# W298/Surtr

Hardware: AMD Instinct MI355X
Metric: fragments/sec (higher is better)
Workload: dtype f32

## Files before the change

### surtr_amd/csrc/prep_sorted.h

```cpp
#pragma once
#include "wave_clip.h"

#define PS_NEVER 0x7Fu
#ifndef SURTR_PS_NB
#define SURTR_PS_NB 896u
#endif
#ifndef SURTR_SPH_FAN
#define SURTR_SPH_FAN 8u
#endif

namespace surtr {

struct SortedRings
{
    const SRow* row_s; const uint32_t* iperm;
    const float4* bsph2; const float4* bsph3;
};

__device__ __forceinline__ uint32_t ps_sphere_fc(const Shared& sh, const uint32_t F, const float4 sp, const uint32_t k0, uint32_t& kstop)
{
    const float mag = fabsf(sp.x) + fabsf(sp.y) + fabsf(sp.z) + sp.w;
    for (uint32_t k = k0; k < F; ++k)
    {
        const float4 mk = sh.pmar[k];
// ... 311 lines not shown
    __syncthreads();
    for (uint32_t id = tid; id < n; id += G)
    {
        const uint32_t v = orig[id] & 0xFFFFu;
        const float4 pr = in.posr_s[orig[id] >> 16];
        T.pos[3 * id] = pr.x; T.pos[3 * id + 1] = pr.y; T.pos[3 * id + 2] = pr.z;
        const uint32_t deg = T.llen[id];
        const int32_t* r = in.nbr + in.loff[v];
        uint16_t* d = T.ring + T.loff[id];
        for (uint32_t j0 = 0; j0 < deg; j0 += 8)
        {
            int32_t u[8];
#pragma unroll
            for (int q = 0; q < 8; ++q) u[q] = (j0 + q < deg) ? r[j0 + q] : -1;
#pragma unroll
            for (int q = 0; q < 8; ++q) if (u[q] >= 0) d[j0 + q] = (uint16_t)ps_newid(bmask, bblk, (uint32_t)u[q], InLds::SENT);
        }
    }
    STAMP(2);
    __syncthreads();
    uint32_t maxb = 0;
    for (uint32_t k = 0; k < F; ++k) maxb = sh.pw[k] > maxb ? sh.pw[k] : maxb;
    maxb_out = maxb;
    T.nS = n; T.nLive = n; T.hUsed = hsum;
}

struct RecLayout { uint32_t hist, zhist, bst, grec, gpos, total; };
__host__ __device__ static inline RecLayout rec_layout(uint32_t F, uint32_t n)
{
    auto up = [](uint32_t b) { return (b + 15u) & ~15u; };
    const uint32_t nn = (n + 15u) & ~15u;
    RecLayout L;
    L.hist = 0; L.zhist = up(4u * F); L.bst = L.zhist + up(4u * F); L.grec = L.bst + up(4u * (F + 2u)); L.gpos = L.grec + 16u * nn;
    L.total = L.gpos + 16u * nn;
    return L;
}

__device__ __attribute__((always_inline)) inline void prepass_emit_records(const SolidIn in, const uint32_t F, Shared& sh, const unsigned long long* bmask, const uint2* bblk,
                                                                           const uint32_t* klist, uint32_t* orig, uint8_t* fcb, uint16_t* sid16, uint32_t* cnt,
                                                                           char* img, const uint32_t n, uint32_t& ncut_out, uint32_t& maxb_out)
{
    const uint32_t tid = threadIdx.x, l = lane_id(), w = wave_id(), G = group_size(), nw = group_waves();
    const RecLayout lay = rec_layout(F, n);
    STAMP_DECL;
    for (uint32_t t = tid; t < n; t += G)
    {
        const uint32_t ke = klist[t], si = ke & 0xFFFFu;
        const uint32_t v = in.perm[si];
        const uint32_t id = ps_newid(bmask, bblk, v, 0u);
        orig[id] = v | (si << 16);
        fcb[id] = (uint8_t)((ke >> 16) & 0x7Fu);
    }
    const uint32_t nsw = nw < 4u ? nw : 4u;
    uint32_t* wcnt = cnt;
    uint32_t* bst = cnt + 4u * (WC_MAXF + 2u);
    for (uint32_t k = tid; k < 4u * (WC_MAXF + 2u); k += G) wcnt[k] = 0u;
    __syncthreads();
    const unsigned long long lt = (1ull << l) - 1ull;
    const uint32_t nb = (n + SURTR_LANES - 1u) >> SURTR_LSH, nbw = (nb + nsw - 1u) / nsw;
    const uint32_t bb0 = w * nbw, bb1 = w < nsw ? (bb0 + nbw < nb ? bb0 + nbw : nb) : bb0;
    for (int pass = 0; pass < 2; ++pass)
    {
        for (uint32_t bb = bb0; bb < bb1; ++bb)
        {
            const uint32_t id = (bb << SURTR_LSH) + l;
            const bool valid = id < n;
            const uint32_t f = valid ? (uint32_t)fcb[id] : 0u;
            const uint32_t bk = (f == PS_NEVER || f > F) ? F : f;
            unsigned long long todo = __ballot(valid);
            uint32_t s = 0;
            while (todo)
            {
                const uint32_t leader = (uint32_t)__builtin_ctzll(todo);
                const uint32_t k0 = lane_bcast(bk, leader);
                const unsigned long long same = __ballot(valid && bk == k0);
                uint32_t base = 0;
                if (l == leader) { base = wcnt[w * (WC_MAXF + 2u) + k0]; wcnt[w * (WC_MAXF + 2u) + k0] = base + wc_popc64(same); }
                base = lane_bcast(base, leader);
                if (valid && bk == k0) s = base + wc_popc64(same & lt);
                todo &= ~same;
            }
            if (valid && pass == 1) sid16[id] = (uint16_t)s;
        }
        if (pass == 1) break;
        __syncthreads();
        if (w == 0u)
        {
            uint32_t carry = 0;
            for (uint32_t k0 = 0; k0 <= F; k0 += SURTR_LANES)
            {
                const uint32_t k = k0 + l;
                uint32_t c = 0;
                if (k <= F) for (uint32_t q = 0; q < nsw; ++q) c += wcnt[q * (WC_MAXF + 2u) + k];
                const uint32_t inc = wave_incl_scan2(make_uint2(c, 0u)).x;
                if (k <= F)
                {
                    uint32_t at = carry + inc - c;
                    bst[k] = at;
                    for (uint32_t q = 0; q < nsw; ++q) { const uint32_t cq = wcnt[q * (WC_MAXF + 2u) + k]; wcnt[q * (WC_MAXF + 2u) + k] = at; at += cq; }
                }
                carry += lane_bcast(inc, SURTR_LANES - 1u);
            }
            if (l == 0u) bst[F + 1u] = carry;
        }
        __syncthreads();
    }
    __syncthreads();
    STAMP(2);
    WcW4* grec = (WcW4*)(img + lay.grec);
    float4* gpos = (float4*)(img + lay.gpos);
    for (uint32_t id = tid; id < n; id += G)
    {
        const uint32_t vi = orig[id], v = vi & 0xFFFFu;
        const uint32_t f = fcb[id];
        const uint32_t len = in.llen[v];
        const int32_t* r = in.nbr + in.loff[v];
        const uint32_t s = sid16[id];
        const float4 pr = in.posr_s[vi >> 16];
        int32_t u[7]; uint32_t e[7];
#pragma unroll
        for (uint32_t q = 0; q < 7u; ++q) u[q] = r[q < len ? q : 0u];
#pragma unroll
        for (uint32_t q = 0; q < 7u; ++q) e[q] = ps_newid(bmask, bblk, (uint32_t)u[q], 0xFFFFFFFFu);
#pragma unroll
        for (uint32_t q = 0; q < 7u; ++q) e[q] = q >= len ? WC_NONE : (e[q] == 0xFFFFFFFFu ? WC_SENT : (uint32_t)sid16[e[q]]);
        WcW4 wr;
        wr.a = e[0] | (e[1] << 16); wr.b = e[2] | (e[3] << 16); wr.c = e[4] | (e[5] << 16);
        wr.d = e[6] | (((f == PS_NEVER ? SURTR_NEVER : f) | (len << 8)) << 16);
        grec[s] = wr;
        gpos[s] = make_float4(pr.x, pr.y, pr.z, __uint_as_float(id));
    }
    prepass_finish_hist(F, sh);
    uint32_t* hs = (uint32_t*)(img + lay.hist); uint32_t* zs = (uint32_t*)(img + lay.zhist); uint32_t* bs = (uint32_t*)(img + lay.bst);
    for (uint32_t k = tid; k < F; k += G) { hs[k] = sh.hist[k]; zs[k] = sh.zhist[k]; }
    for (uint32_t k = tid; k <= F + 1u; k += G) bs[k] = bst[k];
    uint32_t ncut = 0, maxb = 0;
    for (uint32_t k = 0; k < F; ++k) { const uint32_t c = bst[k + 1u] - bst[k]; ncut += c != 0u ? 1u : 0u; maxb = c > maxb ? c : maxb; }
    ncut_out = ncut; maxb_out = maxb;
    STAMP(74);
}

template <class LT>
__device__ __attribute__((always_inline)) inline int wc_attach(LT& W, const uint32_t* hist, const uint32_t* zhist, const uint32_t* bst, const uint32_t F, const uint32_t n,
                                                               unsigned long long& zmask, WcCtr& ctr, uint32_t* __restrict__ why)
{
    const uint32_t tid = threadIdx.x;
    ctr.ac = 0u; ctr.sc = 0u;
    zmask = 0ull;
    if (F > WC_MAXF || n == 0u || n >= WC_MAXN) WC_RET(1);
    WSTAMP_DECL;
    for (uint32_t k = tid; k < F; k += group_size()) { W.hist[k] = hist[k]; W.zhist[k] = zhist[k]; }
    for (uint32_t k = tid; k <= F + 1u; k += group_size()) W.bst[k] = bst[k];
    if (tid == 0u) { W.zm[0] = 0u; W.zm[1] = 0u; for (int q = 0; q < 6; ++q) (&W.fl[0][0])[q] = 0u; }
    __syncthreads();
    WSTAMP(1);
    WCOUNT(16, 1); WCOUNT(17, n);
    return 0;
}

}
```

### surtr_amd/csrc/surtr_ctx.h

```cpp
#pragma once
#include <algorithm>
#include <chrono>
#include <cstdint>
#include <cstdlib>
#include <string>
#include <vector>

#include "../../include/surtr_hip.h"
#include "clip_core.h"

using namespace surtr;

struct PairRec
{
    uint32_t cv_off, cv_n, ch_off, ch_n;
    uint32_t mv_off, mv_n, mh_off, mh_n;
    uint32_t ni, isl_off;
    uint32_t status;
    uint32_t img_fmt, img_off, img_n, img_h, img_pc;
    uint32_t cv_bad;
};

enum { IMG_NONE = 0,
       IMG_NARROW = 1,
       IMG_WIDE = 2,
       IMG_EMPTY = 3,
       IMG_REC = 4 };

struct ImgLayout { uint32_t hist, zhist, nzero, mask, loff, llen, comp, ring, pos, total; };
__host__ __device__ static inline ImgLayout img_layout(uint32_t F, uint32_t nbV, uint32_t n, uint32_t hsum, uint32_t posCap = 0)
{
    auto up = [](uint32_t b) { return (b + 15u) & ~15u; };
    ImgLayout L;
    L.hist = 0; L.zhist = up(4u * F); L.nzero = L.zhist + up(4u * F); L.mask = L.nzero + up(4u * F); L.loff = L.mask + up(8u * nbV);
    L.llen = L.loff + up(2u * n); L.comp = L.llen + up(n); L.ring = L.comp + up(n); L.pos = L.ring + up(2u * hsum);
    L.total = L.pos + up(12u * (n > posCap ? n : posCap));
    return L;
}

struct ImgArena { char* base; uint32_t cap16; };

struct PrepPool { char* base; size_t per_wg; uint32_t VMAX; };
static size_t prep_bytes_per_wg(uint32_t VMAX)
{
    auto r = [](size_t b) { return (b + 255) & ~(size_t)255; };
    return 2 * r((size_t)VMAX * 4) + r((size_t)(VMAX / SURTR_SB + 2) * 4) + 2 * r((size_t)(VMAX / SURTR_LANES + 2) * 8) +
           2 * r((size_t)VMAX + 64) +
           2 * r((size_t)VMAX * 4) +
           r((size_t)VMAX * 2 + 64);
}

struct FragRec
{
    int32_t cell, piece, island;
    uint32_t mv_off, mv_n, mh_off, mh_n;
    uint32_t cv_off, cv_n, ch_off, ch_n;
    uint32_t idx_off, idx_n;
    uint32_t o_mv, o_mh, o_cv, o_ch, o_idx;
};

struct Arena
{
    float* pos; uint32_t* loff; uint32_t* llen; int32_t* nbr; uint32_t* idx;
    uint2* isl;
    uint32_t capV, capH, capI, capIsl;
    uint32_t* cursors;
};

enum : uint32_t
{
    CUR_V = 0,
    CUR_H = 1,
    CUR_I = 2,
    CUR_ISL = 3,
    CUR_Q_CLIP = 4,
    CUR_STATUS = 5,
    CUR_Q_REFIT = 6,
    CUR_Q_FACES = 7,
    CUR_Q_CONVEX = 8,
    CUR_Q_PREP = 9,
    CUR_IMG = 10,
    CUR_Q_BIG = 11,
    CUR_Q_HALF = 12,
    CUR_Q_RETRY = 13,
    CUR_FLAGGED_FRAGS = 14,
    CUR_FLAGGED_PAIRS = 15,
    CUR_CLS_CLIP = 16,
    CUR_CLS_FRAG = 32,
    CUR_CLS_PREP = 48,
    CUR_CLS_HALF = 64,
    CUR_RETRY_N = CUR_CLS_HALF,
    CUR_CVX_RESUMED = 78,
    CUR_REFIT_RESUMED = 79,
    CUR_CVX_TOOK = 80,
    CUR_REFIT_TOOK = 82,
    CUR_BIG_QUOTA = 84,
    CUR_FACES2_N = 85,
    CUR_Q_FACES2 = 86,
    CUR_CVX_GAVE_UP = 87,
    CUR_REC_TOOK = 88,
    CUR_REC_HANDED = 89,
    CUR_LIT_TOO_LARGE = 90,
    CUR_REC_IMAGES = 91,
    CUR_SORTED_SEL = 92,
    CUR_REC_SPENT = 93,
    CUR_CATCH_CLIPPED = 94,
    CUR_UNREFITTED = 95,
    CUR_WC_WHY = 96,
    CUR_Q_CONVEX2 = 125,
    CUR_STATS_WORDS = 128,
    CUR_HO_PUSHED = 146,
    CUR_HO_STARTED = 147,
    CUR_HO_SIGNED_OFF = 148,
    CUR_HO_POLL_SLOT = 149,
    CUR_Q_CATCH = 150,
    CUR_Q_SWEEP = 151,
    CUR_HO_WORDS = 6,
    CUR_COUNT = 256
};
static_assert(CUR_V == 0 && CUR_H == 1 && CUR_I == 2 && CUR_ISL == 3 && CUR_STATUS == 5 && CUR_CLS_CLIP == 16 && CUR_CLS_FRAG == 32 &&
              CUR_CLS_PREP == 48 && CUR_CLS_HALF == 64 && CUR_REC_TOOK == 88 && CUR_REC_HANDED == 89 && CUR_LIT_TOO_LARGE == 90 &&
              CUR_UNREFITTED == 95 && CUR_WC_WHY == 96, "include/surtr_hip.h publishes these slots of surtr_queue_stats by number");
static_assert(CUR_STATS_WORDS <= CUR_COUNT && CUR_Q_SWEEP + 1 == CUR_HO_PUSHED + CUR_HO_WORDS && CUR_HO_PUSHED + CUR_HO_WORDS <= CUR_COUNT &&
              CUR_Q_FACES2 == CUR_FACES2_N + 1, "slot map");

struct alignas(16) SRow { uint32_t w[4]; };

struct Pieces
{
    const float* mpos; const uint32_t* mloff; const uint32_t* mllen; const int32_t* mnbr; const uint32_t* mvo; const uint8_t* mtri; const float* mrad;
    const uint32_t* mperm; const float4* mposr_s; const float4* mbsph; const uint32_t* mbo;
    const float* cpos; const uint32_t* cloff; const uint32_t* cllen; const int32_t* cnbr; const uint32_t* cvo; const uint8_t* ctri; const float* crad;
    const uint32_t* cperm; const float4* cposr_s; const float4* cbsph; const uint32_t* cbo;
    uint32_t n;
    const uint8_t* mdup; const uint8_t* cdup;
    const SRow* mrow_s; const uint32_t* miperm;
    const float4* mbsph2; const uint32_t* mbo2; const float4* mbsph3; const uint32_t* mbo3;
};

struct ScratchPool
{
    char* base; size_t per_wg;
    uint32_t CV, CH, VMAX;
};

struct Scratch
{
    float* pos;
    uint32_t* g_loff; uint32_t* g_llen; int8_t* g_comp; uint32_t* g_ring;
    uint32_t* g_succ; uint32_t* g_pred; uint32_t* g_pcnt;
    uint32_t* aux0; uint32_t* aux1; uint32_t* aux2; uint32_t* aux3;
    int8_t* g_gcomp;
    uint2* blk;
    unsigned long long* gmask; uint2* gblk;
    float* t_pos; uint32_t* t_loff; uint32_t* t_llen; int8_t* t_comp; uint32_t* t_ring;
    uint32_t CV, CH;
};

__device__ static Scratch carve(const ScratchPool& P, uint32_t wg)
{
    Scratch S;
    char* p = P.base + (size_t)wg * P.per_wg;
    auto take = [&](size_t bytes) { char* r = p; p += (bytes + 255) & ~(size_t)255; return r; };
    S.pos = (float*)take((size_t)P.CV * 12);
    S.g_loff = (uint32_t*)take((size_t)P.CV * 4);
    S.g_llen = (uint32_t*)take((size_t)P.CV * 4);
    S.g_comp = (int8_t*)take((size_t)P.CV);
    S.g_ring = (uint32_t*)take((size_t)P.CH * 4);
    S.g_succ = (uint32_t*)take((size_t)P.CV * 4);
    S.g_pred = (uint32_t*)take((size_t)P.CV * 4);
    S.g_pcnt = (uint32_t*)take((size_t)P.CV * 4);
    const size_t AV = P.CV > P.VMAX ? P.CV : P.VMAX;
    S.aux0 = (uint32_t*)take(AV * 4);
    S.aux1 = (uint32_t*)take((size_t)P.CV * 4);
    S.aux2 = (uint32_t*)take(AV * 4);
    S.aux3 = (uint32_t*)take((size_t)P.CV * 4);
    S.g_gcomp = (int8_t*)take((size_t)P.CV);
    S.blk = (uint2*)take((size_t)(P.CV / SURTR_LANES + 4) * 8);
    S.gmask = (unsigned long long*)take((size_t)(P.VMAX / SURTR_LANES + 2) * 8);
    S.gblk = (uint2*)take((size_t)(P.VMAX / SURTR_LANES + 2) * 8);
    S.t_pos = (float*)take((size_t)P.CV * 12); S.t_loff = (uint32_t*)take((size_t)P.CV * 4); S.t_llen = (uint32_t*)take((size_t)P.CV * 4);
    S.t_comp = (int8_t*)take((size_t)P.CV); S.t_ring = (uint32_t*)take((size_t)P.CH * 4);
    S.CV = P.CV; S.CH = P.CH;
    return S;
}

static size_t scratch_bytes_per_wg(uint32_t CV, uint32_t CH, uint32_t VMAX)
{
    auto r = [](size_t b) { return (b + 255) & ~(size_t)255; };
    return 2 * r((size_t)CV * 12) + 9 * r((size_t)CV * 4) + 2 * r((size_t)std::max(CV, VMAX) * 4) + 3 * r((size_t)CV) + 2 * r((size_t)CH * 4) + r((size_t)(CV / SURTR_LANES + 4) * 8) +
           2 * r((size_t)(VMAX / SURTR_LANES + 2) * 8);
}

struct FaceScratch
{
    int32_t* base; size_t per_wg; uint32_t HF;
};

struct surtr_ctx;

template <class T>
struct DevBuf
{
    T* p = nullptr;
    size_t cap = 0;
    DevBuf() = default;
    DevBuf(DevBuf&& o) noexcept : p(o.p), cap(o.cap) { o.p = nullptr; o.cap = 0; }
    DevBuf& operator=(DevBuf&& o) noexcept { if (this != &o) { reset(); p = o.p; cap = o.cap; o.p = nullptr; o.cap = 0; } return *this; }
    ~DevBuf() { reset(); }
    void reset() { if (p) (void)hipFree(p); p = nullptr; cap = 0; }
    operator T*() const { return p; }
    int grow(surtr_ctx* ctx, size_t need, size_t alloc = 0);
};

struct PieceSet
{
    DevBuf<float> pos; DevBuf<uint32_t> loff, llen; DevBuf<int32_t> nbr; DevBuf<uint32_t> vo; DevBuf<uint8_t> tri; DevBuf<float> rad;
    DevBuf<uint32_t> perm; DevBuf<float4> posr_s, bsph; DevBuf<uint32_t> bo;
    DevBuf<float> box; DevBuf<unsigned long long> key, key2; DevBuf<uint32_t> val;
    DevBuf<uint8_t> dup;
    DevBuf<uint32_t> iperm; DevBuf<SRow> row_s;
    DevBuf<float4> bsph2; DevBuf<uint32_t> bo2; DevBuf<float4> bsph3; DevBuf<uint32_t> bo3;
};

struct CellBuffers
{
    DevBuf<double> seeds; DevBuf<uint32_t> goff; DevBuf<char> slots; DevBuf<uint32_t> cfo, cvo;
    DevBuf<int32_t> gen; DevBuf<uint32_t> fvo; DevBuf<double> verts; DevBuf<uint32_t> heads;
    uint32_t n = 0, nf = 0, nfv = 0;
};

#define SURTR_LVS (SURTR_LV / 2u)
#define SURTR_LHS ((SURTR_LH * 11u / 24u) & ~7u)
#ifndef SURTR_HALF_ROOM
#define SURTR_HALF_ROOM 2u
#endif
__host__ __device__ static inline bool fits_half(uint32_t n, uint32_t h, uint32_t capVs) { return SURTR_HALF_ROOM * n <= capVs && SURTR_HALF_ROOM * h <= SURTR_LHS; }
static inline bool surtr_fits_half(uint32_t n, uint32_t h) { return fits_half(n, h, SURTR_LVS); }

struct surtr_ctx
{
    int device = 0;
    bool frags_of_pieces = false;
    uint32_t hw_wg = 512, hw_wg_faces = 1024, hw_wg_prep = 1792, hw_wg_big = 48, budget_vmax = 0xFFFFFFFFu, budget_hmax = 0xFFFFFFFFu;
    uint32_t max_wg = 512, max_wg_faces = 1024, max_wg_small = 2048, max_wg_lean = 3072, max_wg_prep = 1792, max_wg_half = 1024;
    DevBuf<uint32_t> d_hlist;
    uint32_t vmin = 0;
    ScratchPool pool_half{}; uint32_t n_wg_half = 0; DevBuf<char> pool_half_buf;
    bool half_on = false;
    PrepPool prep{nullptr, 0, 0}; uint32_t n_wg_prep = 0; DevBuf<char> prep_buf;
    ImgArena img{nullptr, 0}; DevBuf<char> img_buf;
    DevBuf<uint32_t> d_order;
    DevBuf<uint32_t> d_forder;
    bool wave_big = false;
    uint32_t n_wg_big = 48;
    hipStream_t stream2 = nullptr;
    hipStream_t stream3 = nullptr;
    hipEvent_t ev_prep = nullptr, ev_big = nullptr, ev_half = nullptr, ev_cvx = nullptr;
    uint32_t events_in_flight = 1;
    hipStream_t stream = nullptr;
    std::string err;
    uint32_t n_pieces = 0, vmax = 0, hmax = 0, cvmax = 0, chmax = 0;
// ... 252 lines not shown
```

### surtr_amd/csrc/surtr_hip.hip

```cpp
#include <algorithm>
#include <cmath>
#include <cstdio>
#include <cstdlib>
#include <cstring>
#include <string>
#include <type_traits>
#include <vector>

#include "surtr_ctx.h"
#include "small_clip.h"
#ifndef SC_RESUME
#define SC_RESUME 1
#endif
#include "literal_clip.h"
#include "wave_clip.h"
#include "prep_sorted.h"

template <uint32_t LV, uint32_t LH>
struct alignas(16) LdsTopoT
{
    static_assert(LV % 16 == 0 && LH % 8 == 0, "clip_image copies 16-byte words into these arrays");
    static constexpr uint32_t kLV = LV, kLH = LH;
    alignas(16) uint16_t loff[LV];
    alignas(16) uint8_t llen[LV];
// ... 1121 lines not shown
        }
        __syncthreads();
    }
    if (err == 0 && !gone) err = clip_global(min, F, S, sh, consume);
    __syncthreads();
    return finish_pair(A, pairs, p, rec, err);
}

template <bool HALF = false, class LT>
__device__ __attribute__((always_inline)) static inline void clip_pair_general(Shared& sh, LT& L, Scratch& S, const ScratchPool& pool, uint32_t wg, const Pieces& P,
                                       const float4* __restrict__ planes, const uint32_t* __restrict__ plane_off, uint32_t cell_begin,
                                       const Arena& A, const ImgArena& IA, PairRec* __restrict__ pairs, const uint2* __restrict__ pair_list,
                                       uint32_t* __restrict__ horder, const uint32_t p, PairRec rec)
{
    const uint32_t tid = threadIdx.x;
    const PairAt at = pair_where(p, pair_list, cell_begin, P.n);
    const uint32_t cell = at.cell, piece = at.piece;
    const uint32_t f0 = plane_off[cell], F = plane_off[cell + 1] - f0;
    for (uint32_t k = tid; k < F; k += group_size()) sh.planes[k] = planes[f0 + k];
    __syncthreads();
    SolidIn min = mesh_solid_in(P, piece);
    auto consume = [&](auto& T) -> int {
        if (T.nLive == 0) return 0;
        return park_mesh_islands(T, sh, A, rec);
    };
    if (P.mdup[piece] != 0 && min.nv <= SURTR_LITERAL_START_V)
    {
        if (HALF) { if (tid == 0) horder[atomicAdd(&A.cursors[CUR_RETRY_N], 1u)] = p; }
        else pair_global(P, piece, F, pool, wg, A, &sh, pairs, p, 1u);
        return;
    }
    int err;
    if (HALF)
    {
        if (rec.img_fmt == IMG_NARROW) err = clip_image<false>(IA.base + (size_t)rec.img_off * 16u, rec.img_n, rec.img_h, 0u, min, F, S, sh, L, consume);
        else err = clip_any<false>(min, F, S, sh, L, consume);
        __syncthreads();
        if (err == SURTR_OVERFLOW)
        {
            if (tid == 0) horder[atomicAdd(&A.cursors[CUR_RETRY_N], 1u)] = p;
            return;
        }
    }
    else
    {
        err = SURTR_OVERFLOW;
        if (rec.img_fmt == IMG_NARROW) err = clip_image<false>(IA.base + (size_t)rec.img_off * 16u, rec.img_n, rec.img_h, rec.img_pc, min, F, S, sh, L, consume);
        else if (rec.img_fmt != IMG_WIDE) err = clip_any<false>(min, F, S, sh, L, consume);
        __syncthreads();
        if (err == SURTR_OVERFLOW)
        {
            pair_global(P, piece, F, pool, wg, A, &sh, pairs, p, 0u);
            return;
        }
    }
    if (err == SURTR_E_TOPOLOGY && min.nv <= SURTR_LITERAL_MESH_V)
    {
        __syncthreads();
        if (HALF) { if (tid == 0) horder[atomicAdd(&A.cursors[CUR_RETRY_N], 1u)] = p; }
        else pair_global(P, piece, F, pool, wg, A, &sh, pairs, p, 1u);
        return;
    }
    finish_pair(A, pairs, p, rec, err);
}

template <bool HALF = false, class LT>
__device__ __attribute__((always_inline)) static inline void clip_pairs_body(Shared& sh, LT& L, const ScratchPool& pool, uint32_t wg, const Pieces& P, const float4* __restrict__ planes,
                                       const uint32_t* __restrict__ plane_off, uint32_t cell_begin, uint32_t n_pairs,
                                       const Arena& A, const ImgArena& IA, PairRec* __restrict__ pairs,
                                       const uint2* __restrict__ pair_list, const uint32_t* __restrict__ order,
                                       uint32_t* __restrict__ horder, int cls_hi, int cls_lo, uint32_t qcur)
{
    const uint32_t tid = threadIdx.x;
    Scratch S = carve(pool, wg);
#ifdef SURTR_STAMP
    const unsigned long long wg_t0 = __builtin_readcyclecounter();
#endif
    const int h_hi = HALF ? 6 : (cls_hi < 0 ? 0 : -1), h_lo = cls_hi < 0 ? 0 : 1;
    while (true)
    {
        __syncthreads();
        if (tid == 0)
        {
            uint32_t t = atomicAdd(&A.cursors[qcur], 1u), p = 0xFFFFFFFFu;
            if (!HALF) p = pair_of_ticket(A, order, n_pairs, t, CUR_CLS_CLIP, cls_hi, cls_lo);
            if (p == 0xFFFFFFFFu) p = pair_of_ticket(A, horder, n_pairs, t, CUR_CLS_HALF, h_hi, h_lo);
            sh.misc[7] = p;
        }
        __syncthreads();
        const uint32_t p = sh.misc[7];
        if (p >= n_pairs) break;
        PairRec rec = pairs[p];
        if (rec.cv_n == 0 || rec.status != 0) continue;
        if (rec.img_fmt == IMG_EMPTY) continue;
        if (rec.img_fmt == IMG_REC) rec.img_fmt = IMG_NONE;
#ifdef SURTR_STAMP
        const unsigned long long pair_t0 = __builtin_readcyclecounter();
        if (tid == 0) for (int q = 0; q < 16; ++q) sh.ph[q] = 0;
#endif
        clip_pair_general<HALF>(sh, L, S, pool, wg, P, planes, plane_off, cell_begin, A, IA, pairs, pair_list, horder, p, rec);
#ifdef SURTR_STAMP
        if (tid == 0) { const unsigned long long d = __builtin_readcyclecounter() - pair_t0; int bkt = 0; while ((d >> bkt) > 1 && bkt < 30) ++bkt; bkt = bkt < 16 ? 0 : bkt - 16; if (bkt > 9) bkt = 9; atomicAdd(&g_stamp[(cls_hi == 15 ? 51 : 21) + bkt], 1ull); }
#endif
    }
#ifdef SURTR_STAMP
    if (tid == 0) { const unsigned long long d = __builtin_readcyclecounter() - wg_t0; const int o = cls_hi == 15 ? 48 : 16; atomicAdd(&g_stamp[o], d); atomicMax(&g_stamp[o + 1], d); atomicAdd(&g_stamp[o + 2], 1ull); }
#endif
}

__global__ __launch_bounds__(SURTR_WG) __attribute__((amdgpu_waves_per_eu(2, 4))) void k_clip_pairs(Pieces P, const float4* __restrict__ planes,
                                                         const uint32_t* __restrict__ plane_off, uint32_t cell_begin,
                                                         uint32_t n_pairs,
                                                         ScratchPool pool, Arena A, ImgArena IA, PairRec* __restrict__ pairs,
                                                         const uint2* __restrict__ pair_list, const uint32_t* __restrict__ order,
                                                         uint32_t* __restrict__ horder, int cls_hi, int cls_lo, uint32_t qcur)
{
    __shared__ Shared sh;
    __shared__ LdsTopo L;
    clip_pairs_body(sh, L, pool, blockIdx.x, P, planes, plane_off, cell_begin, n_pairs, A, IA, pairs, pair_list, order, horder, cls_hi, cls_lo, qcur);
}

__global__ __launch_bounds__(SURTR_WGS) __attribute__((amdgpu_waves_per_eu(2, 4))) void k_clip_pairs_half(Pieces P, const float4* __restrict__ planes,
                                                         const uint32_t* __restrict__ plane_off, uint32_t cell_begin,
                                                         uint32_t n_pairs,
                                                         ScratchPool pool, Arena A, ImgArena IA, PairRec* __restrict__ pairs,
                                                         const uint2* __restrict__ pair_list, uint32_t* __restrict__ horder)
{
    __shared__ Shared sh;
    __shared__ LdsTopoHalf L;
    clip_pairs_body<true>(sh, L, pool, blockIdx.x, P, planes, plane_off, cell_begin, n_pairs, A, IA, pairs, pair_list, nullptr, horder, 6, 1, CUR_Q_HALF);
}

__global__ __launch_bounds__(SURTR_WG) void k_clip_pairs_big(Pieces P, const float4* __restrict__ planes,
                                                             const uint32_t* __restrict__ plane_off, uint32_t cell_begin,
                                                             uint32_t n_pairs,
                                                             ScratchPool pool, uint32_t wg_base, Arena A, ImgArena IA,
                                                             PairRec* __restrict__ pairs, const uint2* __restrict__ pair_list,
                                                             const uint32_t* __restrict__ order)
{
    __shared__ Shared sh;
    __shared__ LdsTopoBig L;
    clip_pairs_body(sh, L, pool, wg_base + blockIdx.x, P, planes, plane_off, cell_begin, n_pairs, A, IA, pairs, pair_list, order, nullptr, 15, 14, CUR_Q_BIG);
}

struct GenLds { Shared sh; LdsTopo L; };
struct GenLdsBig { Shared sh; LdsTopoBig L; };
template <class WL, class GL, bool FALLBACK = true, bool OLD_IMAGES = FALLBACK>
__device__ __attribute__((always_inline)) static inline void clip_pairs_wave_body(unsigned char* lds_raw, uint32_t wg, const Pieces& P, const float4* __restrict__ planes,
                                                         const uint32_t* __restrict__ plane_off, uint32_t cell_begin,
                                                         uint32_t n_pairs,
                                                         const ScratchPool& pool, const Arena& A, const ImgArena& IA, PairRec* __restrict__ pairs,
                                                         const uint2* __restrict__ pair_list, const uint32_t* __restrict__ order,
                                                         uint32_t* __restrict__ horder, int cls_hi, int cls_lo, uint32_t qcur, uint32_t walk0,
                                                         uint32_t* __restrict__ hlist, uint32_t cbase)
{
    WL& W = *reinterpret_cast<WL*>(lds_raw);
    GL& Gn = *reinterpret_cast<GL*>(lds_raw);
    const uint32_t tid = threadIdx.x;
    char* slot = pool.base + (size_t)wg * pool.per_wg;
    Scratch S{};
    if (FALLBACK) S = carve(pool, wg);
    if (!FALLBACK && tid == 0) atomicAdd(&A.cursors[CUR_HO_STARTED], 1u);
    while (true)
    {
        __syncthreads();
        if (tid == 0)
        {
            W.misc[7] = take_pair(A, order, n_pairs, qcur, cbase, cls_hi, cls_lo);
        }
        __syncthreads();
        const uint32_t p = W.misc[7];
        if (p >= n_pairs) break;
        PairRec rec = pairs[p];
        if (rec.cv_n == 0 || rec.status != 0) continue;
        if (rec.img_fmt == IMG_EMPTY) continue;
        const PairAt at = pair_where(p, pair_list, cell_begin, P.n);
        const uint32_t cell = at.cell, piece = at.piece;
        const uint32_t f0 = plane_off[cell], F = plane_off[cell + 1] - f0;
        int err = WC_BAIL;
        if ((rec.img_fmt == IMG_NARROW || rec.img_fmt == IMG_REC) && P.mdup[piece] == 0 && F <= WC_MAXF)
        {
            for (uint32_t k = tid; k < F; k += group_size()) W.planes[k] = planes[f0 + k];
            const uint32_t m0 = P.mvo[piece], V = P.mvo[piece + 1] - m0;
            const uint32_t nbV = (V + SURTR_LANES - 1u) >> SURTR_LSH;
            char* img = IA.base + (size_t)rec.img_off * 16u;
            unsigned long long zmask = 0ull;
            WcOut o{0u, 0u, 0u, 0u};
            WcCtr ctr{0u, 0u};
#ifdef SURTR_STAMP
            if (tid == 0) for (int q = 0; q < 32; ++q) W.ph[q] = 0ull;
#endif
            bool fits = false;
            WcGlob g;
            if (rec.img_fmt == IMG_REC)
            {
                const RecLayout rl = rec_layout(F, rec.img_n);
                g.grec = (WcW4*)(img + rl.grec); g.gpos = (float4*)(img + rl.gpos); g.cpos = (float4*)slot;
                fits = 16u * (size_t)(2u * WL::kNR) <= pool.per_wg;
                if (fits) err = wc_attach(W, (const uint32_t*)(img + rl.hist), (const uint32_t*)(img + rl.zhist), (const uint32_t*)(img + rl.bst), F, rec.img_n, zmask, ctr, A.cursors + CUR_WC_WHY);
            }
            else if constexpr (OLD_IMAGES)
            {
                const ImgLayout lay = img_layout(F, nbV, rec.img_n, rec.img_h);
                const WcImg im{(const uint16_t*)(img + lay.loff), (const uint8_t*)(img + lay.llen), (const uint8_t*)(img + lay.comp),
                               (const uint16_t*)(img + lay.ring), (const float*)(img + lay.pos), (const uint32_t*)(img + lay.hist),
                               (const uint32_t*)(img + lay.zhist), (const uint32_t*)(img + lay.nzero), rec.img_n, rec.img_h};
                g = wc_glob(slot, pool.per_wg, rec.img_n, 2u * WL::kNR, fits);
                if (fits) err = wc_load(W, im, F, g, zmask, ctr, A.cursors + CUR_WC_WHY);
            }
            if (err == 0) err = wc_planes(W, F, rec.img_n, V - rec.img_n, zmask, g, 2u * WL::kNR, o, ctr, A.cursors + CUR_WC_WHY, walk0);
            if (err == 0 && o.nLive != 0u) err = wc_park(W, F, rec.img_n, o, g, A, rec, ctr, A.cursors + CUR_WC_WHY);
#ifdef SURTR_STAMP
            __syncthreads();
            if (tid == 0)
            {
                for (int q = 0; q < 29; ++q) if (q != 22 && q != 23 && W.ph[q]) atomicAdd(&g_wstamp[q], W.ph[q]);
                if (p < 8192u)
                {
                    uint32_t mb = 0; for (uint32_t k = 0; k < F; ++k) { const uint32_t c = W.bst[k + 1u] - W.bst[k]; mb = c > mb ? c : mb; }
                    g_wneed[4u * p] = rec.img_n; g_wneed[4u * p + 1u] = mb; g_wneed[4u * p + 2u] = err == 0 ? (uint32_t)W.ph[31] : 0xFFFFFFFFu;
                    unsigned long long cyc = 0; for (int q = 0; q < 16; ++q) cyc += W.ph[q];
                    g_wneed[4u * p + 3u] = (uint32_t)cyc;
                }
                if (err == 0)
                {
                    unsigned long long c = W.ph[31] / 4096ull, c2 = W.ph[29] / 4096ull;
                    atomicAdd(&g_wstamp[32 + (int)(c > 15ull ? 15ull : c)], 1ull);
                    atomicAdd(&g_wstamp[48 + (int)(c2 > 15ull ? 15ull : c2)], 1ull);
                }
            }
#endif
            if (err == WC_BAIL && rec.img_fmt == IMG_REC) { rec.img_fmt = IMG_NONE; if (tid == 0) atomicAdd(&A.cursors[CUR_REC_SPENT], 1u); }
        }
        if (tid == 0) atomicAdd(&A.cursors[err == WC_BAIL ? CUR_REC_HANDED : CUR_REC_TOOK], 1u);
        if (err == WC_BAIL)
        {
            if constexpr (FALLBACK)
            {
                __syncthreads();
                clip_pair_general(Gn.sh, Gn.L, S, pool, wg, P, planes, plane_off, cell_begin, A, IA, pairs, pair_list, horder, p, rec);
            }
            else if (tid == 0)
            {
                pairs[p] = rec;
                __threadfence();
                atomicExch(&hlist[atomicAdd(&A.cursors[CUR_HO_PUSHED], 1u)], p);
            }
            continue;
        }
        finish_pair(A, pairs, p, rec, err);
    }
    if (!FALLBACK && tid == 0) { __threadfence(); atomicAdd(&A.cursors[CUR_HO_SIGNED_OFF], 1u); }
}

__global__ __launch_bounds__(SURTR_WG) __attribute__((amdgpu_waves_per_eu(2, 4))) void k_clip_pairs_wave(Pieces P, const float4* __restrict__ planes,
                                                         const uint32_t* __restrict__ plane_off, uint32_t cell_begin,
                                                         uint32_t n_pairs,
                                                         ScratchPool pool, Arena A, ImgArena IA, PairRec* __restrict__ pairs,
                                                         const uint2* __restrict__ pair_list, const uint32_t* __restrict__ order,
                                                         uint32_t* __restrict__ horder, int cls_hi, int cls_lo, uint32_t qcur, uint32_t walk0)
{
    constexpr size_t kBytes = sizeof(WcLds) > sizeof(GenLds) ? sizeof(WcLds) : sizeof(GenLds);
    __shared__ alignas(16) unsigned char lds_raw[kBytes];
    clip_pairs_wave_body<WcLds, GenLds>(lds_raw, blockIdx.x, P, planes, plane_off, cell_begin, n_pairs, pool, A, IA, pairs, pair_list, order, horder, cls_hi, cls_lo, qcur, walk0, nullptr, CUR_CLS_CLIP);
}

#ifndef SURTR_MAIN_THREADS
#define SURTR_MAIN_THREADS (2u * SURTR_WG)
#endif
#ifndef SURTR_CATCH_POLL
#define SURTR_CATCH_POLL 8u
#endif
#define SURTR_CATCH_WG_MAX 32u
#ifndef SURTR_WR_MAIN
#define SURTR_WR_MAIN 3072u
#define SURTR_WNL_MAIN 3584u
#endif
typedef WcLdsT<SURTR_WR_MAIN, SURTR_WNL_MAIN, (SURTR_MAIN_THREADS / SURTR_LANES > SURTR_NWAVE ? SURTR_MAIN_THREADS / SURTR_LANES : SURTR_NWAVE), true> WcLdsMain;
__global__ __launch_bounds__(SURTR_MAIN_THREADS) __attribute__((amdgpu_waves_per_eu(SURTR_MAIN_THREADS > SURTR_WG ? 4 : 2, 4))) void k_clip_pairs_main(Pieces P, const float4* __restrict__ planes,
                                                         const uint32_t* __restrict__ plane_off, uint32_t cell_begin,
                                                         uint32_t n_pairs,
                                                         ScratchPool pool, Arena A, ImgArena IA, PairRec* __restrict__ pairs,
                                                         const uint2* __restrict__ pair_list, const uint32_t* __restrict__ order,
                                                         uint32_t* __restrict__ hlist, uint32_t walk0)
{
    __shared__ alignas(16) unsigned char lds_raw[sizeof(WcLdsMain)];
    clip_pairs_wave_body<WcLdsMain, WcLdsMain, false, true>(lds_raw, blockIdx.x, P, planes, plane_off, cell_begin, n_pairs, pool, A, IA, pairs, pair_list, order, nullptr, 11, 0, CUR_Q_CLIP, walk0, hlist, CUR_CLS_CLIP);
}

#define SURTR_H_TAKEN 0xFFFFFFFEu
__global__ __launch_bounds__(SURTR_WG) __attribute__((amdgpu_waves_per_eu(2, 4))) void k_clip_pairs_catch(Pieces P, const float4* __restrict__ planes,
                                                         const uint32_t* __restrict__ plane_off, uint32_t cell_begin,
                                                         uint32_t n_pairs,
                                                         ScratchPool pool, uint32_t wg_base, Arena A, ImgArena IA, PairRec* __restrict__ pairs,
                                                         const uint2* __restrict__ pair_list, const uint32_t* __restrict__ order,
                                                         uint32_t* __restrict__ hlist, uint32_t hcap, uint32_t n_main, uint32_t sweep, uint32_t n_poll)
{
    __shared__ Shared sh;
    __shared__ LdsTopo L;
    const uint32_t tid = threadIdx.x, wg = wg_base + blockIdx.x;
    Scratch S = carve(pool, wg);
    bool own = sweep == 0u;
    while (true)
    {
        __syncthreads();
        if (tid == 0)
        {
            uint32_t p = 0xFFFFFFFFu;
            if (sweep != 0u)
            {
                const uint32_t pushed = A.cursors[CUR_HO_PUSHED] < hcap ? A.cursors[CUR_HO_PUSHED] : hcap;
                for (uint32_t t = atomicAdd(&A.cursors[CUR_Q_SWEEP], 1u); t < pushed; t = atomicAdd(&A.cursors[CUR_Q_SWEEP], 1u))
                {
                    const uint32_t v = atomicExch(&hlist[t], SURTR_H_TAKEN);
                    if (v < n_pairs) { p = v; break; }
                }
            }
            else if (own)
            {
                p = take_pair(A, order, n_pairs, CUR_Q_CATCH, CUR_CLS_CLIP, 13, 12);
            }
            if (sweep == 0u && p == 0xFFFFFFFFu && n_poll != 0u && (own ? blockIdx.x : 0u) < n_poll)
            {
                own = false;
                const uint32_t t = atomicAdd(&A.cursors[CUR_HO_POLL_SLOT], 1u);
                for (uint32_t spin = 0; t < hcap; ++spin)
                {
                    const uint32_t v = atomicAdd(&hlist[t], 0u);
                    if (v < n_pairs) { atomicExch(&hlist[t], SURTR_H_TAKEN); p = v; break; }
                    if (atomicAdd(&A.cursors[CUR_HO_SIGNED_OFF], 0u) >= n_main && atomicAdd(&A.cursors[CUR_HO_PUSHED], 0u) <= t) break;
                    if (spin > (1u << 12) && atomicAdd(&A.cursors[CUR_HO_STARTED], 0u) == 0u) break;
                    if (spin > (1u << 22)) break;
                    __builtin_amdgcn_s_sleep(32);
                }
            }
            sh.misc[7] = p;
            sh.misc[6] = own ? 1u : 0u;
        }
        __syncthreads();
        const uint32_t p = sh.misc[7];
        own = sh.misc[6] != 0u;
        if (p >= n_pairs) break;
        PairRec rec = pairs[p];
        if (rec.cv_n == 0 || rec.status != 0) continue;
        if (rec.img_fmt == IMG_EMPTY) continue;
        if (rec.img_fmt == IMG_REC) rec.img_fmt = IMG_NONE;
        if (tid == 0) atomicAdd(&A.cursors[CUR_CATCH_CLIPPED], 1u);
        clip_pair_general(sh, L, S, pool, wg, P, planes, plane_off, cell_begin, A, IA, pairs, pair_list, (uint32_t*)nullptr, p, rec);
    }
}

__global__ __launch_bounds__(SURTR_WG) void k_clip_pairs_wave_big(Pieces P, const float4* __restrict__ planes,
                                                         const uint32_t* __restrict__ plane_off, uint32_t cell_begin,
                                                         uint32_t n_pairs,
                                                         ScratchPool pool, uint32_t wg_base, Arena A, ImgArena IA, PairRec* __restrict__ pairs,
                                                         const uint2* __restrict__ pair_list, const uint32_t* __restrict__ order,
                                                         int cls_hi, int cls_lo, uint32_t qcur, uint32_t walk0)
{
    constexpr size_t kBytes = sizeof(WcLdsBig) > sizeof(GenLdsBig) ? sizeof(WcLdsBig) : sizeof(GenLdsBig);
    __shared__ alignas(16) unsigned char lds_raw[kBytes];
    clip_pairs_wave_body<WcLdsBig, GenLdsBig>(lds_raw, wg_base + blockIdx.x, P, planes, plane_off, cell_begin, n_pairs, pool, A, IA, pairs, pair_list, order, nullptr, cls_hi, cls_lo, qcur, walk0, nullptr, CUR_CLS_CLIP);
}

__global__ __launch_bounds__(SURTR_WG_WIDE) void k_frag_table(const PairRec* __restrict__ pairs, uint32_t n_pairs,
                                                         uint32_t n_pieces, uint32_t cell_begin, Arena A,
                                                         uint2* __restrict__ blk, FragRec* __restrict__ frags,
                                                         uint32_t cap_frags, surtr_counts* __restrict__ counts,
                                                         const uint2* __restrict__ pair_list, uint32_t* __restrict__ forder)
{
    __shared__ Shared sh;
    for (uint32_t q = threadIdx.x; q < 16u; q += group_size()) sh.hist[q] = 0;
    auto fn = [&](uint32_t p) -> uint2 { return make_uint2(pairs[p].ni, 0u); };
    uint32_t nf = 0, dum = 0;
    scan_blocks(n_pairs, blk, sh, fn, nf, dum);
    const uint32_t nb = (n_pairs + SURTR_LANES - 1u) >> SURTR_LSH;
    if (nf <= cap_frags)
    {
        for (uint32_t b = wave_id(); b < nb; b += group_waves())
        {
            const uint32_t p = (b << SURTR_LSH) + lane_id();
            uint2 c = make_uint2(0u, 0u);
            if (p < n_pairs) c = fn(p);
            const uint2 e = wave_excl2(c);
            if (p < n_pairs && c.x)
            {
                const PairRec r = pairs[p];
                uint32_t f = blk[b].x + e.x;
                uint32_t vo = r.mv_off, ho = r.mh_off;
                for (uint32_t t = 0; t < r.ni; ++t, ++f)
                {
                    const uint2 is = A.isl[r.isl_off + t];
                    FragRec fr;
                    const PairAt at = pair_where(p, pair_list, cell_begin, n_pieces);
                    fr.cell = (int32_t)at.cell; fr.piece = (int32_t)at.piece; fr.island = (int32_t)t;
                    fr.mv_off = vo; fr.mv_n = is.x; fr.mh_off = ho; fr.mh_n = is.y;
                    fr.cv_off = r.cv_off; fr.cv_n = r.cv_n; fr.ch_off = r.ch_off; fr.ch_n = r.ch_n;
                    fr.idx_off = 0; fr.idx_n = 0; fr.o_mv = fr.o_mh = fr.o_cv = fr.o_ch = fr.o_idx = 0;
                    frags[f] = fr;
                    uint32_t cls = 0; while ((is.x >> (cls + 1u)) != 0u && cls < 15u) ++cls;
                    forder[(size_t)cls * cap_frags + atomicAdd(&sh.hist[cls], 1u)] = f;
                    vo += is.x; ho += is.y;
                }
            }
        }
    }
    __syncthreads();
    for (uint32_t q = threadIdx.x; q < 16u; q += group_size()) A.cursors[CUR_CLS_FRAG + q] = sh.hist[q];
    if (threadIdx.x == 0)
    {
        counts->n_frag = nf <= cap_frags ? nf : 0u;
        counts->n_pairs = n_pairs;
        if (nf > cap_frags) atomicMax(&A.cursors[CUR_STATUS], (uint32_t)SURTR_E_CAPACITY);
    }
}

__device__ static uint32_t frag_of_ticket(const Arena& A, const uint32_t* __restrict__ forder, uint32_t cap_frags, uint32_t t)
{
    for (int cls = 15; cls >= 0; --cls)
    {
        const uint32_t cnt = A.cursors[CUR_CLS_FRAG + cls];
        if (t < cnt) return forder[(size_t)cls * cap_frags + t];
        t -= cnt;
    }
    return 0xFFFFFFFFu;
}

struct ArgF { float v; uint32_t i; };
struct ArgD { double v; uint32_t i; };

template <class T, class A>
__device__ static A wg_argmax(A mine, A* slots )
{
    auto step = [&](auto mv) {
        A o = mv(mine);
        if (o.i != 0xFFFFFFFFu && (mine.i == 0xFFFFFFFFu || o.v > mine.v || (o.v == mine.v && o.i < mine.i))) mine = o;
    };
    auto mover = [](auto ctrl_tag, auto mask_tag) {
        return [](A a) {
            constexpr int CTRL = decltype(ctrl_tag)::value, MASK = decltype(mask_tag)::value;
            A o;
// ... 1759 lines not shown
    if (ctx->pool.base && ctx->pool.CV >= CV && ctx->pool.CH >= CH && ctx->pool.VMAX >= VMAX && ctx->n_wg >= n_wg && ctx->n_wg_faces_alloc >= n_wg_faces) return SURTR_OK;
    free_scratch(ctx);
    int rc = alloc_pool(ctx, ctx->pool_buf, ctx->pool, ctx->n_wg, CV, CH, VMAX, n_wg);
    const uint32_t HF_full = need_h + need_h / 2 + 8192;
    uint32_t tier = SURTR_FACES_TIER_DEFAULT;
    if (ctx->events_in_flight > 1u) tier /= 4u;
    if (const char* e = getenv("SURTR_FACES_TIER_HE")) { const long v = atol(e); if (v >= 64) tier = (uint32_t)v; }
    FaceScratch fs{nullptr, 0, std::min(HF_full, tier)};
    fs.per_wg = (size_t)12 * fs.HF;
    const uint32_t blk_per_wg = fs.HF / SURTR_LANES + 4;
    if (rc == SURTR_OK) rc = ctx->fs_buf.grow(ctx, fs.per_wg * n_wg_faces);
    if (rc == SURTR_OK) rc = ctx->d_blk.grow(ctx, (size_t)blk_per_wg * n_wg_faces);
    FaceScratch fs_big{}; uint32_t n_wg_big = 0, blk_per_wg_big = 0;
    if (rc == SURTR_OK && HF_full > fs.HF)
    {
        size_t free_b = 0, total_b = 0;
        if (hipMemGetInfo(&free_b, &total_b) != hipSuccess || total_b == 0) total_b = (size_t)64 << 30;
        if (const char* e = getenv("SURTR_MEM_BUDGET_MB")) { const long v = atol(e); if (v > 0) total_b = (size_t)v << 20; }
        fs_big.HF = HF_full; fs_big.per_wg = (size_t)12 * HF_full;
        n_wg_big = (uint32_t)std::min<size_t>(64, std::max<size_t>(2, (total_b / 16) / (fs_big.per_wg * 4)));
        blk_per_wg_big = HF_full / SURTR_LANES + 4;
        rc = ctx->fs_big_buf.grow(ctx, fs_big.per_wg * n_wg_big);
        if (rc == SURTR_OK) rc = ctx->d_blk_big.grow(ctx, (size_t)blk_per_wg_big * n_wg_big);
    }
    if (rc) { free_scratch(ctx); return rc; }
    fs.base = ctx->fs_buf; fs_big.base = ctx->fs_big_buf;
    ctx->fs = fs; ctx->blk_per_wg = blk_per_wg; ctx->n_wg_faces_alloc = n_wg_faces;
    ctx->fs_big = fs_big; ctx->blk_per_wg_big = blk_per_wg_big; ctx->n_wg_faces_big = n_wg_big;
    return SURTR_OK;
}

static int ensure_scratch_small(surtr_ctx* ctx, uint32_t n_wg)
{
    const uint32_t need_v = 2 * ctx->cvmax + 4 * SURTR_MAXF + 256, need_h = 2 * ctx->chmax + 12 * SURTR_MAXF + 1024;
    const uint32_t CV = 2 * need_v + 1024, CH = 3 * need_h + 4096, VMAX = need_v;
    if (ctx->pool_small.base && ctx->pool_small.CV >= CV && ctx->pool_small.CH >= CH && ctx->n_wg_small >= n_wg) return SURTR_OK;
    return alloc_pool(ctx, ctx->pool_small_buf, ctx->pool_small, ctx->n_wg_small, CV, CH, VMAX, n_wg);
}

static int ensure_scratch_half(surtr_ctx* ctx, uint32_t n_wg)
{
    if (ctx->pool_half.base && ctx->n_wg_half >= n_wg) return SURTR_OK;
    return alloc_pool(ctx, ctx->pool_half_buf, ctx->pool_half, ctx->n_wg_half, SURTR_LVS + 256u, SURTR_LHS + 256u, SURTR_LVS + 64u, n_wg);
}

static int ensure_prep(surtr_ctx* ctx, uint32_t n_pairs, uint32_t n_wg)
{
    const uint32_t VMAX = std::max(ctx->vmax, 64u);
    if (!(ctx->prep.base && ctx->prep.VMAX >= VMAX && ctx->n_wg_prep >= n_wg))
    {
        ctx->prep = PrepPool{nullptr, 0, 0}; ctx->n_wg_prep = 0;
        ctx->prep_buf.reset();
        const size_t per_wg = prep_bytes_per_wg(VMAX);
        const int rc = ctx->prep_buf.grow(ctx, per_wg * n_wg);
        if (rc) return rc;
        ctx->prep = PrepPool{ctx->prep_buf, per_wg, VMAX}; ctx->n_wg_prep = n_wg;
    }
    int rc = ctx->d_order.grow(ctx, (size_t)n_pairs * 64);
    if (rc) return rc;
    const uint64_t full = (uint64_t)ctx->vmax * 16 + (uint64_t)ctx->hmax * 2;
    const uint64_t lds = (uint64_t)SURTR_LV * 16 + (uint64_t)SURTR_LH * 2;
    const uint64_t per_pair = std::min(full, lds) + ctx->vmax / 8 + 2048;
    uint64_t bytes = std::min<uint64_t>(std::max<uint64_t>((uint64_t)n_pairs * per_pair, 1ull << 20), 4ull << 30);
    if (const char* e = getenv("SURTR_IMG_BYTES")) { const long long v = atoll(e); if (v >= 4096) bytes = (uint64_t)v; }
    const uint32_t cap16 = (uint32_t)(bytes / 16);
    if (!(ctx->img.base && ctx->img.cap16 >= cap16) || (getenv("SURTR_IMG_BYTES") && ctx->img.cap16 != cap16))
    {
        ctx->img = ImgArena{nullptr, 0};
        ctx->img_buf.reset();
        rc = ctx->img_buf.grow(ctx, (size_t)cap16 * 16);
        if (rc) return rc;
        ctx->img = ImgArena{ctx->img_buf, cap16};
    }
    return SURTR_OK;
}

static void free_arena(surtr_ctx* ctx)
{
    auto& B = ctx->arena_buf;
    B.pos.reset(); B.loff.reset(); B.llen.reset(); B.nbr.reset(); B.idx.reset(); B.isl.reset();
    ctx->d_frags.reset(); ctx->d_forder.reset(); ctx->d_frag_status.reset(); ctx->d_face_list.reset();
    ctx->arena = Arena{}; ctx->arena.cursors = B.cursors; ctx->cap_frags = 0;
}

static uint32_t refit_planes(const surtr_ctx* ctx) { return std::min(2u * RH_MAXFACE, 2u * (3u * ctx->refit_limit - 8u)); }

static int ensure_arena(surtr_ctx* ctx, uint32_t n_pairs, uint64_t min_v = 0, uint64_t min_h = 0, uint64_t min_i = 0)
{
    const uint64_t xp = refit_planes(ctx) - 8u;
    uint64_t av = ctx->user_av ? ctx->user_av : std::max<uint64_t>(std::max<uint64_t>((uint64_t)ctx->vmax * 8, ctx->tot_mv * 3) + (uint64_t)n_pairs * (256 + 8 * xp), 1u << 16);
    uint64_t ah = ctx->user_ah ? ctx->user_ah : std::max<uint64_t>(std::max<uint64_t>((uint64_t)ctx->hmax * 8, ctx->tot_mh * 3) + (uint64_t)n_pairs * (1024 + 32 * xp), 1u << 18);
    uint64_t ai = ctx->user_ai ? ctx->user_ai : ah * 2;
    av = std::max(av, min_v); ah = std::max(ah, min_h); ai = std::max(ai, min_i);
    av = std::min<uint64_t>(av, 0xFFFFFFF0ull); ah = std::min<uint64_t>(ah, 0xFFFFFFF0ull); ai = std::min<uint64_t>(ai, 0xFFFFFFF0ull);
    const uint32_t capIsl = (uint32_t)std::min<uint64_t>((uint64_t)n_pairs * 4 + 1024, 0x7FFFFFFFull);
    if (!(ctx->arena.pos && ctx->arena.capV >= av && ctx->arena.capH >= ah && ctx->arena.capI >= ai && ctx->arena.capIsl >= capIsl))
    {
        free_arena(ctx);
        auto& B = ctx->arena_buf;
        int rc = B.pos.grow(ctx, av * 3);
        if (rc == SURTR_OK) rc = B.loff.grow(ctx, av);
        if (rc == SURTR_OK) rc = B.llen.grow(ctx, av);
        if (rc == SURTR_OK) rc = B.nbr.grow(ctx, ah);
        if (rc == SURTR_OK) rc = B.idx.grow(ctx, ai);
        if (rc == SURTR_OK) rc = B.isl.grow(ctx, capIsl);
        if (rc == SURTR_OK) rc = ctx->d_frags.grow(ctx, capIsl);
        if (rc == SURTR_OK) rc = ctx->d_forder.grow(ctx, (size_t)capIsl * 16);
        if (rc == SURTR_OK) rc = ctx->d_frag_status.grow(ctx, capIsl);
        if (rc == SURTR_OK) rc = ctx->d_face_list.grow(ctx, capIsl);
        if (rc) { free_arena(ctx); return rc; }
        ctx->arena = Arena{B.pos, B.loff, B.llen, B.nbr, B.idx, B.isl, (uint32_t)av, (uint32_t)ah, (uint32_t)ai, capIsl, B.cursors};
        ctx->cap_frags = capIsl;
    }
    int rc = ctx->d_pairs.grow(ctx, n_pairs);
    if (rc == SURTR_OK) rc = ctx->d_cvx_giveup.grow(ctx, n_pairs);
    if (rc) return rc;
    return ctx->d_scanblk.grow(ctx, std::max(n_pairs, ctx->cap_frags) / SURTR_LANES + 4);
}

__global__ void k_event_init(uint32_t* __restrict__ cursors, uint32_t* __restrict__ counts, uint32_t n_counts, uint32_t* __restrict__ frag_status,
                             uint32_t n_status, uint32_t* __restrict__ hlist, uint32_t n_hlist)
{
    const uint32_t i0 = blockIdx.x * blockDim.x + threadIdx.x, step = gridDim.x * blockDim.x;
    for (uint32_t i = i0; i < CUR_COUNT; i += step) cursors[i] = 0u;
    for (uint32_t i = i0; i < n_counts; i += step) counts[i] = 0u;
    for (uint32_t i = i0; i < n_status; i += step) frag_status[i] = 0u;
    for (uint32_t i = i0; i < n_hlist; i += step) hlist[i] = 0xFFFFFFFFu;
}

static int upload_pair_order(surtr_ctx* ctx, const uint32_t* ord, uint32_t n_pairs)
{
    const int rc = ctx->d_pair_order.grow(ctx, n_pairs);
    if (rc) return rc;
    HIPCHK(hipStreamSynchronize(ctx->stream));
    HIPCHK(hipMemcpyAsync(ctx->d_pair_order, ord, (size_t)n_pairs * 4, hipMemcpyHostToDevice, ctx->stream));
    HIPCHK(hipStreamSynchronize(ctx->stream));
    return SURTR_OK;
}

#ifndef SURTR_REC_MAXN
#define SURTR_REC_MAXN 2304u
#endif
#ifndef SURTR_FRONT_PAR_MAX
#define SURTR_FRONT_PAR_MAX 1024u
#endif
struct EventPlan
{
    bool cell_order;
    decltype(&k_prep_pairs) prep;
    uint32_t prep_threads;
    bool wave_on, split_on, use_half, front_par, both;
    bool cvx_lean;
    uint32_t rec_on;
    uint32_t big_quota, big_n, walk0, n_catch, n_poll;
    uint32_t n_wg, n_wg_cvx, n_wg_lean, n_wg_cvx2, n_wg_prep, n_wg_big, n_wg_half, n_wg_retry, n_wg_sweep;
    uint32_t g_refit, g_faces, t_faces;
    hipStream_t st_cvx, st_main, st_bigk, st_refit;
};

static EventPlan plan_event(const surtr_ctx* ctx, uint32_t n_pairs, bool pair_list, uint32_t flags)
{
    EventPlan pl{};
    const uint32_t n1 = std::max(n_pairs, 1u), max_wg = ctx->max_wg;
    pl.cell_order = !pair_list && n_pairs && ctx->n_pieces && n_pairs % ctx->n_pieces == 0 && !getenv("SURTR_NO_CELL_ORDER");
    pl.n_wg = std::max(1u, std::min(n1, max_wg));
    pl.n_wg_cvx = std::max(1u, std::min(n1, ctx->max_wg_small));
    pl.n_wg_lean = std::max(1u, std::min(n1, ctx->max_wg_lean));
    pl.n_wg_cvx2 = std::min(n1, 64u);
    pl.n_wg_half = std::max(1u, std::min(n1, ctx->max_wg_half));
    pl.n_wg_prep = std::max(1u, std::min(n1, ctx->max_wg_prep));
    pl.n_wg_big = std::min(ctx->n_wg_big, n1);
    pl.n_wg_retry = std::min(pl.n_wg, 64u);
    pl.big_quota = ctx->wave_big ? 0xFFFFFFFFu : 2u * ctx->n_wg_big;
    if (const char* e = getenv("SURTR_BIG_QUOTA")) pl.big_quota = (uint32_t)atoi(e);
    pl.big_n = (ctx->wave_big && ctx->vmax < 180000u) ? 2800u : 0xFFFFFFFFu;
    const bool half_forced = getenv("SURTR_HALF") != nullptr && atoi(getenv("SURTR_HALF")) != 0;
    const bool many = ctx->events_in_flight > 1u && !half_forced;
    pl.wave_on = 2u * n_pairs > 3u * max_wg || (!half_forced && ctx->vmin >= SURTR_PREP_MINV && ctx->vmax <= 4u * SURTR_REC_MAXN) ||
                 (many && ctx->vmin >= SURTR_PREP_MINV && ctx->vmax <= ctx->prep.VMAX);
    if (const char* e = getenv("SURTR_WAVE")) pl.wave_on = atoi(e) != 0;
    pl.rec_on = pl.wave_on ? 1u : 0u;
    if (const char* e = getenv("SURTR_REC")) pl.rec_on = (pl.wave_on && atoi(e) != 0) ? 1u : 0u;
    if (const char* e = getenv("SURTR_PREP_SORTED")) { if (atoi(e) == 0) pl.rec_on = 2u; }
    uint32_t rec_maxn = SURTR_REC_MAXN;
    if (const char* e = getenv("SURTR_REC_MAXN")) rec_maxn = (uint32_t)atoi(e);
    pl.rec_on |= (rec_maxn < 0xFFFFFFu ? rec_maxn : 0xFFFFFFu) << 8;
    pl.split_on = pl.wave_on && ctx->vmin >= SURTR_PREP_MINV && ctx->vmax <= ctx->prep.VMAX;
    if (const char* e = getenv("SURTR_SPLIT")) pl.split_on = pl.split_on && atoi(e) != 0;
    pl.use_half = ctx->half_on && (!pl.split_on || half_forced);
    pl.n_catch = std::min(SURTR_CATCH_WG_MAX, n1);
    pl.n_wg_sweep = std::min(pl.n_catch, SURTR_CATCH_POLL);
    pl.n_poll = ctx->events_in_flight > 1u ? 2u : SURTR_CATCH_POLL;
    if (const char* e = getenv("SURTR_CATCH_POLL")) { const int v = atoi(e); if (v >= 0 && v <= 1024) pl.n_poll = (uint32_t)v; }
    uint32_t wide_max = 4u * ctx->max_wg;
    if (const char* e = getenv("SURTR_PREP_WIDE_MAX")) wide_max = (uint32_t)atoi(e);
    const bool prep_wide = n_pairs != 0 && n_pairs <= wide_max && ctx->vmax >= 8192u && !many;
    pl.front_par = n_pairs != 0 && n_pairs <= SURTR_FRONT_PAR_MAX && !prep_wide;
    if (const char* e = getenv("SURTR_FRONT_PAR")) pl.front_par = n_pairs != 0 && atoi(e) != 0;
    if (pl.front_par) pl.rec_on |= 4u;
    pl.cvx_lean = n_pairs > ctx->max_wg_small;
    if (const char* e = getenv("SURTR_CVX_LEAN")) pl.cvx_lean = n_pairs != 0 && atoi(e) != 0;
    pl.prep = nullptr; pl.prep_threads = SURTR_WG;
    if (n_pairs && prep_wide) { pl.prep = k_prep_pairs_wide; pl.prep_threads = SURTR_WG_WIDE; }
    else if (n_pairs && !(pl.rec_on & 2u) && ctx->vmax < 0xFFFFu && ctx->vmin >= SURTR_PREP_MINV && (ctx->vmax + SURTR_LANES - 1u) / SURTR_LANES <= SURTR_PREP_NB)
        pl.prep = k_prep_pairs_sorted;
    else if (n_pairs) pl.prep = k_prep_pairs;
    pl.walk0 = SURTR_WWALK0;
    if (const char* e = getenv("SURTR_WWALK0")) { const int v = atoi(e); if (v >= 0 && v <= 64) pl.walk0 = (uint32_t)v; }
    pl.st_cvx = pl.front_par ? ctx->stream3 : ctx->stream;
    pl.st_main = pl.front_par ? ctx->stream : ctx->stream2;
    pl.st_bigk = pl.front_par ? ctx->stream2 : ctx->stream;
    pl.both = (flags & SURTR_EVT_REFIT) && (flags & SURTR_EVT_RENDER);
    pl.st_refit = pl.both ? ctx->stream2 : ctx->stream;
    pl.g_refit = ctx->n_wg_small;
    if (pl.both) pl.g_refit = std::min(pl.g_refit, ctx->max_wg_faces / 4u * 5u);
    if (pl.both) if (const char* e = getenv("SURTR_REFIT_WG_BOTH")) { const uint32_t v = (uint32_t)atoi(e); if (v > 0 && v <= ctx->n_wg_small) pl.g_refit = v; }
    pl.g_faces = std::max(1u, ctx->max_wg_faces); pl.t_faces = SURTR_WG;
    if (pl.both) pl.g_faces = std::max(1u, ctx->max_wg_faces / 2u);
    if (pl.both) if (const char* e = getenv("SURTR_FACES_WG_BOTH")) { const uint32_t v = (uint32_t)atoi(e); if (v > 0 && v <= ctx->n_wg_faces_alloc) pl.g_faces = v; }
    if (const char* e = getenv("SURTR_FACES_WG")) { const uint32_t v = (uint32_t)atoi(e); if (v > 0 && v <= ctx->n_wg_faces_alloc) pl.g_faces = v; }
    if (const char* e = getenv("SURTR_FACES_THREADS")) { const uint32_t v = (uint32_t)atoi(e); if (v == 64 || v == 128 || v == 256) pl.t_faces = v; }
    return pl;
}

static int ensure_hull_ws(surtr_ctx* ctx)
{
    if (ctx->refit_limit <= 4u || ctx->d_hull_ws.cap >= 2 * (size_t)ctx->arena.capV) return SURTR_OK;
    HIPCHK(hipStreamSynchronize(ctx->stream));
    return ctx->d_hull_ws.grow(ctx, 2 * (size_t)ctx->arena.capV);
}

static void launch_refit(surtr_ctx* ctx, uint32_t grid, hipStream_t st, bool of_pieces)
{
    const float* cpos = of_pieces ? (const float*)ctx->cset.pos : (const float*)nullptr;
    const uint32_t* cvo = of_pieces ? (const uint32_t*)ctx->cset.vo : (const uint32_t*)nullptr;
    if (ctx->refit_limit <= 4u)
        hipLaunchKernelGGL(k_refit, dim3(grid), dim3(SURTR_LANES), 0, st, ctx->d_frags, ctx->d_counts, ctx->pool_small, ctx->arena, ctx->d_forder, ctx->cap_frags, ctx->d_frag_status,
                           cpos, cvo);
    else
        hipLaunchKernelGGL(k_refit_n, dim3(grid), dim3(SURTR_LANES), 0, st, ctx->d_frags, ctx->d_counts, ctx->pool_small, ctx->arena, ctx->d_forder, ctx->cap_frags, ctx->d_frag_status,
                           cpos, cvo, ctx->refit_limit, (uint32_t*)ctx->d_hull_ws);
}

static int launch_event(surtr_ctx* ctx, uint32_t cell_begin, uint32_t n_pairs, const uint2* d_pair_list, const uint8_t* outside, uint32_t flags)
{
    (void)hipSetDevice(ctx->device);
    budget_workgroups(ctx);
    const uint32_t max_wg = ctx->max_wg, n1 = std::max(n_pairs, 1u);
    int rc = ensure_scratch(ctx, ctx->vmax, ctx->hmax, max_wg + ctx->n_wg_big + SURTR_CATCH_WG_MAX);
    if (rc) return rc;
    rc = ensure_scratch_small(ctx, std::max(ctx->max_wg_small, ctx->n_wg_small));
    if (rc) return rc;
    rc = ensure_scratch_half(ctx, std::max(ctx->max_wg_half, ctx->n_wg_half));
    if (rc) return rc;
    rc = ensure_arena(ctx, n1);
    if (rc) return rc;
    if (flags & SURTR_EVT_REFIT) { rc = ensure_hull_ws(ctx); if (rc) return rc; }
    rc = ensure_prep(ctx, n1, std::max(std::max(1u, std::min(n1, ctx->max_wg_prep)), ctx->n_wg_prep));
    if (rc) return rc;
    hipStream_t st = ctx->stream, st2 = ctx->stream2, st3 = ctx->stream3;
    const uint32_t hcap = n_pairs + 4096u;
    if (ctx->d_hlist.cap < hcap)
    {
        HIPCHK(hipStreamSynchronize(st));
        rc = ctx->d_hlist.grow(ctx, hcap);
        if (rc) return rc;
    }
    const EventPlan pl = plan_event(ctx, n_pairs, d_pair_list != nullptr, flags);
    static_assert(sizeof(surtr_counts) % 4 == 0, "surtr_counts is cleared by words");
    hipLaunchKernelGGL(k_event_init, dim3(SURTR_LANES == 1 ? 1 : 64), dim3(SURTR_LANES == 1 ? 1 : 256), 0, st, ctx->arena.cursors, (uint32_t*)ctx->d_counts.p,
                       (uint32_t)(sizeof(surtr_counts) / 4), ctx->d_frag_status, ctx->cap_frags, ctx->d_hlist, hcap);
    const uint8_t* d_out = nullptr;
    ctx->last_outside.clear();
    if (outside) ctx->last_outside.assign(outside, outside + ctx->n_pieces);
    if (outside)
    {
        HIPCHK(hipMemcpyAsync(ctx->d_outside, outside, ctx->n_pieces, hipMemcpyHostToDevice, st));
        d_out = ctx->d_outside;
    }
    const PieceSet& M = ctx->mset; const PieceSet& C = ctx->cset;
    Pieces P{M.pos, M.loff, M.llen, M.nbr, M.vo, M.tri, M.rad, M.perm, M.posr_s, M.bsph, M.bo,
             C.pos, C.loff, C.llen, C.nbr, C.vo, C.tri, C.rad, C.perm, C.posr_s, C.bsph, C.bo, ctx->n_pieces, M.dup, C.dup,
             M.row_s, M.iperm, M.bsph2, M.bo2, M.bsph3, M.bo3};
    for (int i = 0; i < 16; ++i) ctx->ev_valid[i] = false;
    const uint32_t* d_pair_order = nullptr;
    if (d_pair_list && ctx->pair_order_is_list && ctx->pair_order_count == n_pairs) d_pair_order = ctx->d_pair_order;
    else if (pl.cell_order)
    {
        const uint32_t np = ctx->n_pieces, nc = n_pairs / np;
        if (ctx->pair_order_is_list || ctx->pair_order_begin != cell_begin || ctx->pair_order_count != n_pairs)
        {
            std::vector<uint32_t> cells(nc), ord((size_t)n_pairs);
            for (uint32_t i = 0; i < nc; ++i) cells[i] = i;
            const std::vector<uint32_t>& po = ctx->h_plane_off;
            std::stable_sort(cells.begin(), cells.end(), [&](uint32_t a, uint32_t b) {
                return po[cell_begin + a + 1] - po[cell_begin + a] > po[cell_begin + b + 1] - po[cell_begin + b]; });
            for (uint32_t i = 0; i < nc; ++i) for (uint32_t q = 0; q < np; ++q) ord[(size_t)i * np + q] = cells[i] * np + q;
            int rc2 = upload_pair_order(ctx, ord.data(), n_pairs);
            if (rc2) return rc2;
            ctx->pair_order_is_list = false; ctx->pair_order_begin = cell_begin; ctx->pair_order_count = n_pairs;
        }
        d_pair_order = ctx->d_pair_order;
    }
    uint32_t* const order = ctx->d_order;
    const size_t cap_order = ctx->d_order.cap / 64;
    uint32_t* const porder = ctx->d_order + 16 * cap_order;
    uint32_t* const horder = ctx->d_order + 32 * cap_order;
    const bool wave = n_pairs && pl.wave_on, split = wave && pl.split_on;

    if (pl.front_par)
    {
        HIPCHK(hipEventRecord(ctx->ev_prep, st));
        HIPCHK(hipStreamWaitEvent(pl.st_cvx, ctx->ev_prep, 0));
    }
    PROF_BEGIN_ON(6, pl.st_cvx);
    if (n_pairs && pl.cvx_lean)
    {
        uint32_t* const cvx_porder = pl.front_par ? (uint32_t*)nullptr : porder;
        hipLaunchKernelGGL(k_clip_convex_lean, dim3(pl.n_wg_lean), dim3(SURTR_LANES), 0, pl.st_cvx, P, ctx->d_planes, ctx->d_plane_off, cell_begin, n_pairs,
                           d_out, ctx->arena, ctx->d_pairs, d_pair_list, cvx_porder, d_pair_order, pl.front_par ? 1u : 0u, (uint32_t*)ctx->d_cvx_giveup);
        hipLaunchKernelGGL(k_clip_convex, dim3(pl.n_wg_cvx2), dim3(SURTR_LANES), 0, pl.st_cvx, P, ctx->d_planes, ctx->d_plane_off, cell_begin, n_pairs,
                           d_out, ctx->pool_small, ctx->arena, ctx->d_pairs, d_pair_list, cvx_porder, (const uint32_t*)nullptr,
                           pl.front_par ? 1u : 0u, (const uint32_t*)ctx->d_cvx_giveup);
    }
    else if (n_pairs)
        hipLaunchKernelGGL(k_clip_convex, dim3(pl.n_wg_cvx), dim3(SURTR_LANES), 0, pl.st_cvx, P, ctx->d_planes, ctx->d_plane_off, cell_begin, n_pairs,
                           d_out, ctx->pool_small, ctx->arena, ctx->d_pairs, d_pair_list, pl.front_par ? (uint32_t*)nullptr : porder, d_pair_order,
                           pl.front_par ? 1u : 0u, (const uint32_t*)nullptr);
    PROF_END_ON(6, pl.st_cvx);
    if (pl.front_par) HIPCHK(hipEventRecord(ctx->ev_cvx, pl.st_cvx));
    PROF_BEGIN(7);
    if (pl.prep)
        hipLaunchKernelGGL(pl.prep, dim3(pl.n_wg_prep), dim3(pl.prep_threads), 0, st, P, ctx->d_planes, ctx->d_plane_off, cell_begin, n_pairs,
                           ctx->prep, ctx->arena, ctx->img, std::min((uint32_t)SURTR_LV, ctx->pool.CV), std::min((uint32_t)SURTR_LVS, ctx->pool_half.CV),
                           ctx->d_pairs, d_pair_list, order, porder, horder, pl.use_half ? 1u : 0u, pl.big_quota, pl.big_n, pl.rec_on);
    PROF_END(7);
    HIPCHK(hipEventRecord(ctx->ev_prep, st));
    HIPCHK(hipStreamWaitEvent(st2, ctx->ev_prep, 0));
    HIPCHK(hipStreamWaitEvent(st3, ctx->ev_prep, 0));
    if (pl.front_par)
    {
        HIPCHK(hipStreamWaitEvent(st, ctx->ev_cvx, 0));
        HIPCHK(hipStreamWaitEvent(st2, ctx->ev_cvx, 0));
    }
    PROF_BEGIN_ON(8, pl.st_bigk);
    if (n_pairs && ctx->wave_big)
        hipLaunchKernelGGL(k_clip_pairs_wave_big, dim3(pl.n_wg_big), dim3(SURTR_WG), 0, pl.st_bigk, P, ctx->d_planes,
                           ctx->d_plane_off, cell_begin, n_pairs, ctx->pool, max_wg, ctx->arena, ctx->img, ctx->d_pairs, d_pair_list, order, 15, 14, CUR_Q_BIG, pl.walk0);
    else if (n_pairs)
        hipLaunchKernelGGL(k_clip_pairs_big, dim3(pl.n_wg_big), dim3(SURTR_WG), 0, pl.st_bigk, P, ctx->d_planes,
                           ctx->d_plane_off, cell_begin, n_pairs, ctx->pool, max_wg, ctx->arena, ctx->img, ctx->d_pairs, d_pair_list, order);
    PROF_END_ON(8, pl.st_bigk);
    PROF_BEGIN_ON(11, pl.st_main);
    if (wave) PROF_HIST_BEGIN(11, pl.st_main);
    if (split)
        hipLaunchKernelGGL(k_clip_pairs_main, dim3(pl.n_wg), dim3(SURTR_MAIN_THREADS), 0, pl.st_main, P, ctx->d_planes, ctx->d_plane_off, cell_begin, n_pairs,
                           ctx->pool, ctx->arena, ctx->img, ctx->d_pairs, d_pair_list, order, ctx->d_hlist, pl.walk0);
    else if (wave)
        hipLaunchKernelGGL(k_clip_pairs_wave, dim3(pl.n_wg), dim3(SURTR_WG), 0, pl.st_main, P, ctx->d_planes, ctx->d_plane_off, cell_begin, n_pairs,
                           ctx->pool, ctx->arena, ctx->img, ctx->d_pairs, d_pair_list, order, horder, 13, 0, CUR_Q_CLIP, pl.walk0);
    if (wave) PROF_HIST_END(11, pl.st_main);
    PROF_END_ON(11, pl.st_main);
    PROF_BEGIN_ON(0, pl.st_main);
    if (n_pairs && !pl.wave_on)
    {
        PROF_HIST_BEGIN(0, pl.st_main);
        hipLaunchKernelGGL(k_clip_pairs, dim3(pl.n_wg), dim3(SURTR_WG), 0, pl.st_main, P, ctx->d_planes, ctx->d_plane_off, cell_begin, n_pairs,
                           ctx->pool, ctx->arena, ctx->img, ctx->d_pairs, d_pair_list, order, horder, 13, 0, CUR_Q_CLIP);
        PROF_HIST_END(0, pl.st_main);
    }
    PROF_END_ON(0, pl.st_main);
    PROF_BEGIN_ON(13, st3);
    if (split)
        hipLaunchKernelGGL(k_clip_pairs_catch, dim3(pl.n_catch), dim3(SURTR_WG), 0, st3, P, ctx->d_planes, ctx->d_plane_off, cell_begin, n_pairs,
                           ctx->pool, max_wg + ctx->n_wg_big, ctx->arena, ctx->img, ctx->d_pairs, d_pair_list, order, ctx->d_hlist, hcap, pl.n_wg, 0u, pl.n_poll);
    PROF_END_ON(13, st3);
    PROF_BEGIN_ON(9, st3);
    if (n_pairs && pl.use_half)
        hipLaunchKernelGGL(k_clip_pairs_half, dim3(pl.n_wg_half), dim3(SURTR_WGS), 0, st3, P, ctx->d_planes, ctx->d_plane_off, cell_begin, n_pairs,
                           ctx->pool_half, ctx->arena, ctx->img, ctx->d_pairs, d_pair_list, horder);
    PROF_END_ON(9, st3);
    HIPCHK(hipEventRecord(ctx->ev_half, st3));
    HIPCHK(hipStreamWaitEvent(pl.st_main, ctx->ev_half, 0));
    PROF_BEGIN_ON(10, pl.st_main);
    if (n_pairs && pl.use_half)
        hipLaunchKernelGGL(k_clip_pairs, dim3(pl.n_wg_retry), dim3(SURTR_WG), 0, pl.st_main, P, ctx->d_planes, ctx->d_plane_off, cell_begin, n_pairs,
                           ctx->pool, ctx->arena, ctx->img, ctx->d_pairs, d_pair_list, order, horder, -1, 0, CUR_Q_RETRY);
    if (split)
        hipLaunchKernelGGL(k_clip_pairs_catch, dim3(pl.n_wg_sweep), dim3(SURTR_WG), 0, pl.st_main, P, ctx->d_planes, ctx->d_plane_off, cell_begin, n_pairs,
                           ctx->pool, max_wg + ctx->n_wg_big, ctx->arena, ctx->img, ctx->d_pairs, d_pair_list, order, ctx->d_hlist, hcap, pl.n_wg, 1u, 0u);
    PROF_END_ON(10, pl.st_main);
    HIPCHK(hipEventRecord(ctx->ev_big, st2));
    HIPCHK(hipStreamWaitEvent(st, ctx->ev_big, 0));
    PROF_BEGIN(1);
    hipLaunchKernelGGL(k_frag_table, dim3(1), dim3(SURTR_WG_WIDE), 0, st, ctx->d_pairs, n_pairs, ctx->n_pieces, cell_begin, ctx->arena,
                       ctx->d_scanblk, ctx->d_frags, ctx->cap_frags, ctx->d_counts, d_pair_list, ctx->d_forder);
    PROF_END(1);
    if (pl.both)
    {
        HIPCHK(hipEventRecord(ctx->ev_prep, st));
        HIPCHK(hipStreamWaitEvent(pl.st_refit, ctx->ev_prep, 0));
    }
    if (flags & SURTR_EVT_REFIT)
    {
        PROF_BEGIN_ON(2, pl.st_refit);
        launch_refit(ctx, pl.g_refit, pl.st_refit, true);
        PROF_END_ON(2, pl.st_refit);
    }
    if (flags & SURTR_EVT_RENDER)
    {
        PROF_BEGIN(3);
        const bool tiers = ctx->n_wg_faces_big != 0;
        hipLaunchKernelGGL(k_faces, dim3(pl.g_faces), dim3(pl.t_faces), 0, st, ctx->d_frags, ctx->d_counts, ctx->fs, ctx->d_blk,
                           ctx->blk_per_wg, ctx->arena, ctx->d_forder, ctx->cap_frags, 0u, (uint32_t*)nullptr, (uint32_t*)nullptr, (int32_t*)nullptr,
                           ctx->d_frag_status, (const uint32_t*)nullptr, tiers ? ctx->d_face_list : (uint32_t*)nullptr);
        if (tiers)
            hipLaunchKernelGGL(k_faces, dim3(ctx->n_wg_faces_big), dim3(pl.t_faces), 0, st, ctx->d_frags, ctx->d_counts, ctx->fs_big, ctx->d_blk_big,
                               ctx->blk_per_wg_big, ctx->arena, ctx->d_forder, ctx->cap_frags, 0u, (uint32_t*)nullptr, (uint32_t*)nullptr, (int32_t*)nullptr,
                               ctx->d_frag_status, (const uint32_t*)ctx->d_face_list, (uint32_t*)nullptr);
        PROF_END(3);
    }
    if (pl.both)
    {
        HIPCHK(hipEventRecord(ctx->ev_big, st2));
        HIPCHK(hipStreamWaitEvent(st, ctx->ev_big, 0));
    }
    PROF_BEGIN(4);
    hipLaunchKernelGGL(k_out_scan, dim3(1), dim3(SURTR_WG_WIDE), 0, st, ctx->d_frags, ctx->d_scanblk, ctx->d_counts, ctx->arena);
    PROF_END(4);
    HIPCHK(hipGetLastError());
    ctx->have_event = true; ctx->last_flags = flags; ctx->last_current = false; ctx->frags_of_pieces = true;
    ctx->scene_event_compound.clear(); ctx->scene_event_impacts.clear();
    return SURTR_OK;
}

int surtr_fracture_event_async(surtr_ctx* ctx, uint32_t cell_begin, uint32_t cell_end, const uint8_t* outside, uint32_t flags)
{
    if (!ctx) return SURTR_E_INVALID;
    if (!ctx->n_pieces || !ctx->planes_ready) return SURTR_E_STATE;
    if (cell_end > ctx->n_cells || cell_begin > cell_end) return SURTR_E_INVALID;
    return launch_event(ctx, cell_begin, (cell_end - cell_begin) * ctx->n_pieces, nullptr, outside, flags);
}

int surtr_fracture_pairs_async(surtr_ctx* ctx, uint32_t n_pairs, const uint32_t* pair_cell, const uint32_t* pair_piece, uint32_t flags)
{
    return surtr_event_pairs_masked(ctx, n_pairs, pair_cell, pair_piece, nullptr, flags);
}

}

int surtr_event_pairs_masked(surtr_ctx* ctx, uint32_t n_pairs, const uint32_t* pair_cell, const uint32_t* pair_piece, const uint8_t* outside, uint32_t flags)
{
    if (!ctx || (n_pairs && (!pair_cell || !pair_piece))) return SURTR_E_INVALID;
    if (!ctx->n_pieces || !ctx->planes_ready) return SURTR_E_STATE;
    (void)hipSetDevice(ctx->device);
    std::vector<uint2> list(n_pairs);
    for (uint32_t i = 0; i < n_pairs; ++i)
    {
        if (pair_cell[i] >= ctx->n_cells || pair_piece[i] >= ctx->n_pieces) return SURTR_E_INVALID;
        list[i].x = pair_cell[i]; list[i].y = pair_piece[i];
    }
    const int rc = ctx->d_pair_list.grow(ctx, std::max(n_pairs, 1u));
    if (rc) return rc;
    if (n_pairs) HIPCHK(hipMemcpyAsync(ctx->d_pair_list, list.data(), (size_t)n_pairs * sizeof(uint2), hipMemcpyHostToDevice, ctx->stream));
    HIPCHK(hipStreamSynchronize(ctx->stream));
    ctx->pair_order_count = 0;
    if (n_pairs && !getenv("SURTR_NO_CELL_ORDER"))
    {
        const std::vector<uint32_t>& po = ctx->h_plane_off;
        uint32_t start[SURTR_MAXF + 2] = {0};
        for (uint32_t i = 0; i < n_pairs; ++i) ++start[SURTR_MAXF - (po[pair_cell[i] + 1] - po[pair_cell[i]]) + 1];
        for (uint32_t k = 1; k <= SURTR_MAXF + 1; ++k) start[k] += start[k - 1];
        std::vector<uint32_t> ord(n_pairs);
        for (uint32_t i = 0; i < n_pairs; ++i) ord[start[SURTR_MAXF - (po[pair_cell[i] + 1] - po[pair_cell[i]])]++] = i;
        int rc2 = upload_pair_order(ctx, ord.data(), n_pairs);
        if (rc2) return rc2;
        ctx->pair_order_is_list = true; ctx->pair_order_count = n_pairs;
    }
    return launch_event(ctx, 0, n_pairs, ctx->d_pair_list, outside, flags);
}

extern "C" {

int surtr_place_cells_groups_dev(surtr_ctx* ctx, uint32_t n_groups, const uint32_t* group_cell_off, const float* d_scale3, const float* d_shift3)
{
    if (!ctx || !n_groups || !group_cell_off || !d_scale3 || !d_shift3) return SURTR_E_INVALID;
    if (!ctx->d_v012) return SURTR_E_STATE;
    if (group_cell_off[0] != 0 || group_cell_off[n_groups] != ctx->n_cells) return SURTR_E_INVALID;
    (void)hipSetDevice(ctx->device);
    const uint32_t nf = ctx->n_faces;
    std::vector<uint32_t> face_group(std::max(nf, 1u));
    for (uint32_t g = 0; g < n_groups; ++g)
    {
        if (group_cell_off[g + 1] < group_cell_off[g]) return SURTR_E_INVALID;
        for (uint32_t c = group_cell_off[g]; c < group_cell_off[g + 1]; ++c)
            for (uint32_t f = ctx->h_plane_off[c]; f < ctx->h_plane_off[c + 1]; ++f) face_group[f] = g;
    }
    const int rc = ctx->d_face_group.grow(ctx, std::max(nf, 1u), (size_t)nf + nf / 4 + 64);
    if (rc) return rc;
    HIPCHK(hipMemcpyAsync(ctx->d_face_group, face_group.data(), (size_t)nf * 4, hipMemcpyHostToDevice, ctx->stream));
    if (nf)
        hipLaunchKernelGGL(k_place_cells_groups, dim3((nf + 255) / 256), dim3(256), 0, ctx->stream, nf, ctx->d_v012, ctx->d_face_group, d_scale3, d_shift3, ctx->d_planes);
    HIPCHK(hipGetLastError());
    HIPCHK(hipStreamSynchronize(ctx->stream));
    ctx->planes_ready = true;
    return SURTR_OK;
}

int surtr_place_cells_groups(surtr_ctx* ctx, uint32_t n_groups, const uint32_t* group_cell_off, const float* scale3, const float* translate3)
{
// ... 557 lines not shown
```

### surtr_amd/csrc/wave_clip.h

```cpp
#pragma once
#include "clip_core.h"

#ifndef SURTR_WR
#define SURTR_WR 3584u
#endif
#ifndef SURTR_WNL
#define SURTR_WNL 2560u
#endif
#ifndef SURTR_WWALK0
#define SURTR_WWALK0 4u
#endif
#define WC_MAXF 64u
#define WC_MAXN 0x2000u
#define WC_BAIL 102
#define WC_SENT 0xFFFEu
#define WC_NONE 0xFFFFu
#define WC_WHY_WORDS 29u
static_assert(CUR_WC_WHY + WC_WHY_WORDS <= CUR_STATS_WORDS, "the why[] block ends inside what surtr_queue_stats copies out");
#define WC_RET(site) do { if (threadIdx.x == 0u) atomicAdd(&why[site], 1u); SURTR_DBG("record clip: pair handed on at site %d\n", site); return WC_BAIL; } while (0)
#ifdef SURTR_STAMP
__device__ unsigned long long g_wstamp[64];
__device__ unsigned long long g_wplane[32];
__device__ uint32_t g_wneed[4 * 8192];
#define WSTAMP_DECL unsigned long long ws_t0 = __builtin_readcyclecounter(), ws_t1
#define WSTAMP(i) do { if (threadIdx.x == 0u) { ws_t1 = __builtin_readcyclecounter(); W.ph[i] += ws_t1 - ws_t0; ws_t0 = ws_t1; } } while (0)
#define WCOUNT(i, v) do { if (threadIdx.x == 0u) W.ph[i] += (unsigned long long)(v); } while (0)
#else
#define WSTAMP_DECL
#define WSTAMP(i) do { } while (0)
#define WCOUNT(i, v) do { } while (0)
#endif

namespace surtr {

struct alignas(16) WcW4 { uint32_t a, b, c, d; };

__device__ __forceinline__ uint32_t wc_ld16(const unsigned char* B, uint32_t i16) { uint16_t v; __builtin_memcpy(&v, __builtin_assume_aligned(B + 2u * (size_t)i16, 2), 2); return v; }
__device__ __forceinline__ void wc_st16(unsigned char* B, uint32_t i16, uint32_t v) { const uint16_t x = (uint16_t)v; __builtin_memcpy(__builtin_assume_aligned(B + 2u * (size_t)i16, 2), &x, 2); }
__device__ __forceinline__ uint32_t wc_ld32(const unsigned char* B, uint32_t i16) { uint32_t v; __builtin_memcpy(&v, __builtin_assume_aligned(B + 2u * (size_t)i16, 4), 4); return v; }
__device__ __forceinline__ void wc_st32(unsigned char* B, uint32_t i16, uint32_t v) { __builtin_memcpy(__builtin_assume_aligned(B + 2u * (size_t)i16, 4), &v, 4); }
__device__ __forceinline__ uint32_t wc_ld8(const unsigned char* B, uint32_t i8) { return B[i8]; }
__device__ __forceinline__ void wc_st8(unsigned char* B, uint32_t i8, uint32_t v) { B[i8] = (unsigned char)v; }

struct WcRec
{
    uint32_t w0, w1, w2, w3;
    __device__ __forceinline__ uint32_t tail() const { return w3 >> 16; }
    __device__ __forceinline__ uint32_t e(uint32_t q) const
    {
        const uint32_t w = q < 2u ? w0 : (q < 4u ? w1 : (q < 6u ? w2 : w3));
        return (q & 1u) ? (w >> 16) : (w & 0xFFFFu);
    }
    __device__ __forceinline__ uint32_t find(uint32_t who, uint32_t len) const
    {
        const uint32_t x = who | (who << 16);
        const uint32_t d0 = w0 ^ x, d1 = w1 ^ x, d2 = w2 ^ x, d3 = w3 ^ x;
        uint32_t m = 0;
        m |= (d0 & 0xFFFFu) ? 0u : 1u;  m |= (d0 >> 16) ? 0u : 2u;
        m |= (d1 & 0xFFFFu) ? 0u : 4u;  m |= (d1 >> 16) ? 0u : 8u;
        m |= (d2 & 0xFFFFu) ? 0u : 16u; m |= (d2 >> 16) ? 0u : 32u;
        m |= (d3 & 0xFFFFu) ? 0u : 64u;
        m &= (1u << len) - 1u;
        return m ? (uint32_t)__builtin_ctz(m) : len;
    }
};
struct alignas(8) WcW2 { uint32_t a, b; };
__device__ __forceinline__ WcRec wc_rec(const unsigned char* B, uint32_t byte_off, bool cut)
{
    WcW2 lo, hi;
    __builtin_memcpy(&lo, __builtin_assume_aligned(B + byte_off, 8), 8);
    __builtin_memcpy(&hi, __builtin_assume_aligned(B + byte_off + 8u, 8), 8);
    WcRec r;
    r.w0 = lo.a;
    r.w1 = cut ? (lo.b | 0xFFFF0000u) : lo.b;
    r.w2 = cut ? 0xFFFFFFFFu : hi.a;
    r.w3 = cut ? ((lo.b & 0xFFFF0000u) | 0xFFFFu) : hi.b;
    return r;
}

template <uint32_t NR, uint32_t NL = SURTR_WNL, uint32_t NW = SURTR_NWAVE, bool GSTAGE = (NR < SURTR_WR)>
struct alignas(16) WcLdsT
{
    static constexpr uint32_t kNR = NR, kNL = NL;
    static constexpr bool kGStage = GSTAGE;
    alignas(16) unsigned char U[16u * NR];
    float4 planes[WC_MAXF];
    uint16_t nlist[2][NL];
    uint16_t freel[NL];
    uint32_t hist[WC_MAXF + 1], zhist[WC_MAXF + 1];
    uint32_t bst[WC_MAXF + 2];
    uint32_t wcnt[NW][WC_MAXF + 2];
    uint32_t wsum[2][2 * NW];
    uint32_t bsum[2][2u * (4096u / SURTR_LANES)];
    uint32_t fl[3][2];
    uint32_t zm[2];
    uint32_t misc[8];
#ifdef SURTR_STAMP
    unsigned long long ph[32];
#endif
};
typedef WcLdsT<SURTR_WR> WcLds;
#ifndef SURTR_WR_BIG
#define SURTR_WR_BIG 7424u
#define SURTR_WNL_BIG 6144u
#endif
typedef WcLdsT<SURTR_WR_BIG, SURTR_WNL_BIG> WcLdsBig;

struct WcImg
{
    const uint16_t* loff; const uint8_t* llen; const uint8_t* fc; const uint16_t* ring; const float* pos;
    const uint32_t* hist; const uint32_t* zhist; const uint32_t* nzero;
    uint32_t n, hsum;
};
struct WcGlob { WcW4* grec; float4* gpos; float4* cpos; };
__device__ __forceinline__ WcGlob wc_glob(char* slot, size_t slot_bytes, uint32_t n, uint32_t pool, bool& fits)
{
    WcGlob g;
    const size_t nn = ((size_t)n + 15u) & ~(size_t)15u;
    g.grec = (WcW4*)slot; g.gpos = (float4*)(slot + 16u * nn); g.cpos = (float4*)(slot + 32u * nn);
    fits = 32u * nn + 16u * (size_t)pool <= slot_bytes;
    return g;
}

struct WcOut { uint32_t nl, nLive, rtop, cur; };
struct WcCtr { uint32_t ac, sc; };

template <class LT>
__device__ __forceinline__ bool wc_any(LT& W, uint32_t& c, bool pred, uint32_t slot = 0u)
{
    if (threadIdx.x == 0u) { W.fl[(c + 1u) % 3u][0] = 0u; W.fl[(c + 1u) % 3u][1] = 0u; }
    if (pred) W.fl[c % 3u][slot] = 1u;
    __syncthreads();
    const bool r = W.fl[c % 3u][slot] != 0u;
    ++c;
    return r;
}

template <class LT, class C1, class C2, class P>
__device__ __forceinline__ uint2 wc_scan(LT& W, uint32_t& sc, uint32_t N, C1 count1, C2 count2, P place)
{
    const uint32_t lane = lane_id(), w = wave_id(), nw = group_waves();
    const uint32_t nb = (N + SURTR_LANES - 1u) >> SURTR_LSH, nbw = (nb + nw - 1u) / nw;
    const uint32_t b0 = w * nbw, b1 = b0 + nbw < nb ? b0 + nbw : nb;
    uint32_t* ws = W.wsum[sc & 1u];
    ++sc;
    uint2 mine = make_uint2(0u, 0u);
    for (uint32_t b = b0; b < b1; ++b)
    {
        const uint32_t i = (b << SURTR_LSH) + lane;
        if (i < N) { const uint2 c = count1(i); mine.x += c.x; mine.y += c.y; }
    }
    const uint2 inc = wave_incl_scan2(mine);
    if (lane == SURTR_LANES - 1u) { ws[2u * w] = inc.x; ws[2u * w + 1u] = inc.y; }
    __syncthreads();
    uint2 run = make_uint2(0u, 0u), tot = make_uint2(0u, 0u);
    for (uint32_t q = 0; q < nw; ++q)
    {
        const uint32_t a = ws[2u * q], b = ws[2u * q + 1u];
        if (q < w) { run.x += a; run.y += b; }
        tot.x += a; tot.y += b;
    }
    for (uint32_t b = b0; b < b1; ++b)
    {
        const uint32_t i = (b << SURTR_LSH) + lane;
        uint2 c = make_uint2(0u, 0u);
        if (i < N) c = count2(i);
        const uint2 s = wave_incl_scan2(c);
        if (i < N) place(i, run.x + s.x - c.x, run.y + s.y - c.y);
        run.x += lane_bcast(s.x, SURTR_LANES - 1u); run.y += lane_bcast(s.y, SURTR_LANES - 1u);
    }
    return make_uint2(SURTR_UNIFORM(tot.x), SURTR_UNIFORM(tot.y));
}

template <int NC> struct WcScanState { uint32_t b0, b1; uint2 run; uint2 cc[NC]; uint32_t ax[NC]; };
template <int NC, class LT, class C, class M>
__device__ __forceinline__ uint2 wc_scan_count(LT& W, uint32_t& sc, uint32_t N, WcScanState<NC>& st, C count, M mid)
{
    const uint32_t lane = lane_id(), w = wave_id(), nw = group_waves();
    const uint32_t nb = (N + SURTR_LANES - 1u) >> SURTR_LSH, nbw = (nb + nw - 1u) / nw;
    st.b0 = w * nbw; st.b1 = st.b0 + nbw < nb ? st.b0 + nbw : nb;
    uint32_t* ws = W.wsum[sc & 1u];
    ++sc;
    uint2 mine = make_uint2(0u, 0u);
#pragma unroll
    for (int bi = 0; bi < NC; ++bi)
    {
        st.cc[bi] = make_uint2(0u, 0u); st.ax[bi] = 0u;
        const uint32_t i = ((st.b0 + (uint32_t)bi) << SURTR_LSH) + lane;
        if (st.b0 + (uint32_t)bi < st.b1 && i < N) { st.cc[bi] = count(i, st.ax[bi]); mine.x += st.cc[bi].x; mine.y += st.cc[bi].y; }
    }
    for (uint32_t b = st.b0 + (uint32_t)NC; b < st.b1; ++b)
    {
        const uint32_t i = (b << SURTR_LSH) + lane;
        if (i < N) { uint32_t a; const uint2 c = count(i, a); mine.x += c.x; mine.y += c.y; }
    }
    const uint2 inc = wave_incl_scan2(mine);
    if (lane == SURTR_LANES - 1u) { ws[2u * w] = inc.x; ws[2u * w + 1u] = inc.y; }
    mid();
    __syncthreads();
    uint2 run = make_uint2(0u, 0u), tot = make_uint2(0u, 0u);
    for (uint32_t q = 0; q < nw; ++q)
    {
        const uint32_t a = ws[2u * q], b = ws[2u * q + 1u];
        if (q < w) { run.x += a; run.y += b; }
        tot.x += a; tot.y += b;
    }
    st.run = run;
    return make_uint2(SURTR_UNIFORM(tot.x), SURTR_UNIFORM(tot.y));
}
template <int NC, class C, class P>
__device__ __forceinline__ void wc_scan_place(uint32_t N, WcScanState<NC>& st, C count, P place)
{
    const uint32_t lane = lane_id();
    uint2 run = st.run;
#pragma unroll
    for (int bi = 0; bi < NC; ++bi)
    {
        if (st.b0 + (uint32_t)bi >= st.b1) break;
        const uint32_t i = ((st.b0 + (uint32_t)bi) << SURTR_LSH) + lane;
        const uint2 c = st.cc[bi];
        const uint2 s = wave_incl_scan2(c);
        if (i < N) place(i, run.x + s.x - c.x, run.y + s.y - c.y, c, st.ax[bi]);
        run.x += lane_bcast(s.x, SURTR_LANES - 1u); run.y += lane_bcast(s.y, SURTR_LANES - 1u);
    }
    for (uint32_t b = st.b0 + (uint32_t)NC; b < st.b1; ++b)
    {
        const uint32_t i = (b << SURTR_LSH) + lane;
        uint2 c = make_uint2(0u, 0u); uint32_t a = 0u;
        if (i < N) c = count(i, a);
        const uint2 s = wave_incl_scan2(c);
        if (i < N) place(i, run.x + s.x - c.x, run.y + s.y - c.y, c, a);
        run.x += lane_bcast(s.x, SURTR_LANES - 1u); run.y += lane_bcast(s.y, SURTR_LANES - 1u);
    }
}

template <int NC> struct WcRRState { uint2 cc[NC], ss[NC], px; uint32_t ax[NC]; };
template <int NC, class LT, class PF, class C, class M>
__device__ __forceinline__ uint2 wc_rr_count(LT& W, uint32_t& sc, uint32_t N, WcRRState<NC>& st, PF pref, C count, M mid)
{
    const uint32_t lane = lane_id(), w = wave_id(), nw = group_waves();
    const uint32_t nb = (N + SURTR_LANES - 1u) >> SURTR_LSH;
    uint32_t* bs = W.bsum[sc & 1u];
    ++sc;
    WcW4 pf[NC];
#pragma unroll
    for (int bi = 0; bi < NC; ++bi)
    {
        const uint32_t b = w + (uint32_t)bi * nw, i = (b << SURTR_LSH) + lane;
        pf[bi] = WcW4{0u, 0u, 0u, 0u};
        if (b < nb && i < N) pf[bi] = pref(i);
    }
#pragma unroll
    for (int bi = NC - 1; bi >= 0; --bi)
    {
        const uint32_t b = w + (uint32_t)bi * nw, i = (b << SURTR_LSH) + lane;
        st.cc[bi] = make_uint2(0u, 0u); st.ax[bi] = 0u; st.ss[bi] = make_uint2(0u, 0u);
        if (b < nb)
        {
            if (i < N) st.cc[bi] = count(i, st.ax[bi], pf[bi]);
            st.ss[bi] = wave_incl_scan2(st.cc[bi]);
            if (lane == SURTR_LANES - 1u) { bs[2u * b] = st.ss[bi].x; bs[2u * b + 1u] = st.ss[bi].y; }
        }
    }
    for (uint32_t b = w + (uint32_t)NC * nw; b < nb; b += nw)
    {
        const uint32_t i = (b << SURTR_LSH) + lane;
        uint2 c = make_uint2(0u, 0u);
        if (i < N) { uint32_t a; c = count(i, a, pref(i)); }
        const uint2 s2 = wave_incl_scan2(c);
        if (lane == SURTR_LANES - 1u) { bs[2u * b] = s2.x; bs[2u * b + 1u] = s2.y; }
    }
    mid();
    __syncthreads();
    uint2 run = make_uint2(0u, 0u);
    st.px = make_uint2(0u, 0u);
    for (uint32_t c0 = 0; c0 < nb; c0 += SURTR_LANES)
    {
        const uint32_t b = c0 + lane;
        const uint2 v = b < nb ? make_uint2(bs[2u * b], bs[2u * b + 1u]) : make_uint2(0u, 0u);
        const uint2 inc = wave_incl_scan2(v);
        if (SURTR_LANES > 1u) st.px = make_uint2(run.x + inc.x - v.x, run.y + inc.y - v.y);
        else if (b < nb) { bs[2u * b] = run.x + inc.x - v.x; bs[2u * b + 1u] = run.y + inc.y - v.y; }
        run.x += lane_bcast(inc.x, SURTR_LANES - 1u); run.y += lane_bcast(inc.y, SURTR_LANES - 1u);
    }
    return make_uint2(SURTR_UNIFORM(run.x), SURTR_UNIFORM(run.y));
}
template <int NC, class LT>
__device__ __forceinline__ uint2 wc_rr_base(LT& W, const uint32_t* bs, const WcRRState<NC>& st, uint32_t b)
{
    if (SURTR_LANES > 1u) return make_uint2(lane_bcast(st.px.x, b), lane_bcast(st.px.y, b));
    return make_uint2(bs[2u * b], bs[2u * b + 1u]);
}
template <int NC, class LT, class C, class P>
__device__ __forceinline__ void wc_rr_place(LT& W, uint32_t sc_after, uint32_t N, WcRRState<NC>& st, C count, P place)
{
    const uint32_t lane = lane_id(), w = wave_id(), nw = group_waves();
    const uint32_t nb = (N + SURTR_LANES - 1u) >> SURTR_LSH;
    const uint32_t* bs = W.bsum[(sc_after - 1u) & 1u];
#pragma unroll
    for (int bi = 0; bi < NC; ++bi)
    {
        const uint32_t b = w + (uint32_t)bi * nw, i = (b << SURTR_LSH) + lane;
        if (b >= nb) break;
        const uint2 base = wc_rr_base<NC>(W, bs, st, b);
        const uint2 c = st.cc[bi], s2 = st.ss[bi];
        if (i < N) place(i, base.x + s2.x - c.x, base.y + s2.y - c.y, c, st.ax[bi]);
    }
    for (uint32_t b = w + (uint32_t)NC * nw; b < nb; b += nw)
    {
        const uint32_t i = (b << SURTR_LSH) + lane;
        const uint2 base = wc_rr_base<NC>(W, bs, st, b);
        uint2 c = make_uint2(0u, 0u); uint32_t a = 0u;
        if (i < N) c = count(i, a);
        const uint2 s2 = wave_incl_scan2(c);
        if (i < N) place(i, base.x + s2.x - c.x, base.y + s2.y - c.y, c, a);
    }
}

__device__ __forceinline__ uint32_t wc_popc64(unsigned long long m) { return (uint32_t)__builtin_popcountll(m); }

template <class LT>
__device__ __attribute__((always_inline)) inline int wc_load(LT& W, const WcImg im, const uint32_t F, const WcGlob g,
                                                             unsigned long long& zmask, WcCtr& ctr, uint32_t* __restrict__ why)
{
    const uint32_t tid = threadIdx.x, lane = lane_id(), w = wave_id(), nw = group_waves();
    const unsigned long long lt = (1ull << lane) - 1ull;
    unsigned char* B = W.U;
    const uint32_t n = im.n;
    ctr.ac = 0u; ctr.sc = 0u;
    if (F > WC_MAXF || n == 0u || n >= WC_MAXN || n > 8u * LT::kNR) WC_RET(1);
    const uint32_t tmp16 = 0u;
    for (uint32_t k = tid; k < nw * (WC_MAXF + 2u); k += group_size()) (&W.wcnt[0][0])[k] = 0u;
    for (uint32_t k = tid; k < F; k += group_size()) { W.hist[k] = im.hist[k]; W.zhist[k] = im.zhist[k]; }
    if (tid == 0u) { W.zm[0] = 0u; W.zm[1] = 0u; for (int q = 0; q < 6; ++q) (&W.fl[0][0])[q] = 0u; }
    unsigned long long zm = 0ull;
    for (uint32_t k0 = 0; k0 < F; k0 += SURTR_LANES)
    {
        const uint32_t k = k0 + lane;
        zm |= __ballot(k < F && im.nzero[k] != 0u) << k0;
    }
    zmask = zm;
    if (zm != 0ull) WC_RET(17);
    __syncthreads();
    WSTAMP_DECL;
    const uint32_t nb = (n + SURTR_LANES - 1u) >> SURTR_LSH, nbw = (nb + nw - 1u) / nw;
    const uint32_t bb0 = w * nbw, bb1 = bb0 + nbw < nb ? bb0 + nbw : nb;
    bool odd = false;
    for (int pass = 0; pass < 2; ++pass)
    {
        for (uint32_t bb = bb0; bb < bb1; ++bb)
        {
            const uint32_t b = (bb << SURTR_LSH) + lane;
            const bool valid = b < n;
            const uint32_t f = valid ? (uint32_t)im.fc[b] : 0u;
            uint32_t bk = f == SURTR_NEVER ? F : f;
            if (valid && pass == 0 && (bk > F || (uint32_t)im.llen[b] > 7u)) odd = true;
            if (bk > F) bk = F;
            unsigned long long todo = __ballot(valid);
            uint32_t sid = 0;
            while (todo)
            {
                const uint32_t leader = (uint32_t)__builtin_ctzll(todo);
                const uint32_t k0 = lane_bcast(bk, leader);
                const unsigned long long same = __ballot(valid && bk == k0);
                uint32_t base = 0;
                if (lane == leader) { base = W.wcnt[w][k0]; W.wcnt[w][k0] = base + wc_popc64(same); }
                base = lane_bcast(base, leader);
                if (valid && bk == k0) sid = base + wc_popc64(same & lt);
                todo &= ~same;
            }
            if (valid && pass == 1) wc_st16(B, tmp16 + b, sid);
        }
        if (pass == 1) break;
        __syncthreads();
        if (w == 0u)
        {
            uint32_t carry = 0;
            for (uint32_t k0 = 0; k0 <= F; k0 += SURTR_LANES)
            {
                const uint32_t k = k0 + lane;
                uint32_t c = 0;
                if (k <= F) for (uint32_t q = 0; q < nw; ++q) c += W.wcnt[q][k];
                const uint32_t inc = wave_incl_scan2(make_uint2(c, 0u)).x;
                if (k <= F)
                {
                    uint32_t at = carry + inc - c;
                    W.bst[k] = at;
                    for (uint32_t q = 0; q < nw; ++q) { const uint32_t cq = W.wcnt[q][k]; W.wcnt[q][k] = at; at += cq; }
                }
                carry += lane_bcast(inc, SURTR_LANES - 1u);
            }
            if (lane == 0u) W.bst[F + 1u] = carry;
        }
        __syncthreads();
    }
    if (wc_any(W, ctr.ac, odd)) WC_RET(2);
    WSTAMP(0);
    for (uint32_t b = tid; b < n; b += group_size())
    {
        const uint32_t sid = wc_ld16(B, tmp16 + b);
        const uint32_t lo = im.loff[b], len = im.llen[b], f = im.fc[b];
        uint32_t e[7];
#pragma unroll
        for (uint32_t q = 0; q < 7u; ++q) e[q] = im.ring[lo + (q < len ? q : 0u)];
#pragma unroll
        for (uint32_t q = 0; q < 7u; ++q)
        {
            const uint32_t m = wc_ld16(B, tmp16 + (e[q] < n ? e[q] : 0u));
            e[q] = q >= len ? WC_NONE : (e[q] < n ? m : WC_SENT);
        }
        WcW4 wr;
        wr.a = e[0] | (e[1] << 16); wr.b = e[2] | (e[3] << 16); wr.c = e[4] | (e[5] << 16); wr.d = e[6] | ((f | (len << 8)) << 16);
        g.grec[sid] = wr;
        g.gpos[sid] = make_float4(im.pos[3u * b], im.pos[3u * b + 1u], im.pos[3u * b + 2u], 0.f);
    }
    __syncthreads();
    WSTAMP(1);
    WCOUNT(16, 1); WCOUNT(17, n);
    return 0;
}

template <class LT>
__device__ __attribute__((always_inline)) inline int wc_planes(LT& W, const uint32_t F, const uint32_t n, const uint32_t dropTotal, unsigned long long zmask,
                                                               const WcGlob g, const uint32_t capPool, WcOut& out, WcCtr& ctr, uint32_t* __restrict__ why, const uint32_t walk0 = SURTR_WWALK0)
{
    const uint32_t tid = threadIdx.x, G = group_size();
    unsigned char* B = W.U;
    unsigned char* GB = (unsigned char*)g.grec;
    uint32_t rtop = 0, nl = 0, nLive = n, cur = 0, nfree = 0, fhead = 0;
    uint32_t ac = ctr.ac, sc = ctr.sc;
    out.nl = 0; out.nLive = 0; out.rtop = 0; out.cur = 0;
    WSTAMP_DECL;
    for (uint32_t k = 0; k < F; ++k)
    {
#ifdef SURTR_STAMP
        const unsigned long long pl_t0 = __builtin_readcyclecounter();
#endif
        if ((zmask >> k) & 1ull) WC_RET(3);
        const float4 pl = W.planes[k];
        const uint32_t b0 = SURTR_UNIFORM(W.bst[k]), b1 = SURTR_UNIFORM(W.bst[k + 1u]);
        const uint32_t nCo = b1 - b0;
        uint32_t ltop = 8u * LT::kNR;
        auto carve = [&](uint32_t cnt16) -> uint32_t { ltop -= (cnt16 + 7u) & ~7u; return ltop; };
        const uint32_t NI = nCo + nl;
        if (NI > 4095u) WC_RET(6);
        const bool gstage = LT::kGStage && nCo != 0u && 4u * rtop + 8u * nCo + NI + (NI + 1u) / 2u + 7u * NI + 3u * nl + 128u > ltop;
        if (4u * rtop + (gstage ? 0u : 8u * nCo) + NI + (NI + 1u) / 2u + 64u > ltop) WC_RET(4);
        WCOUNT(26, gstage ? 1 : 0);
        const uint32_t stage = gstage ? 0u : carve(8u * nCo) / 8u;
        auto stage_put = [&](uint32_t i, const WcW4& wr) { if (!gstage) __builtin_memcpy(__builtin_assume_aligned(B + 16u * (size_t)(stage + i), 16), &wr, 16); };
        auto rec_of = [&](uint32_t e) -> WcRec {
            if (e >= WC_MAXN) return wc_rec(B, 8u * (e - WC_MAXN), true);
            if (gstage) { const WcW4 wr = g.grec[e]; return WcRec{wr.a, wr.b, wr.c, wr.d}; }
            return wc_rec(B, 16u * (stage + (e - b0)), false);
        };
        auto tail_ld = [&](uint32_t e) -> uint32_t {
            if (e >= WC_MAXN) return wc_ld16(B, 4u * (e - WC_MAXN) + 3u);
            if (gstage) { uint16_t t; __builtin_memcpy(&t, GB + 16u * (size_t)e + 14u, 2); return t; }
            return wc_ld16(B, 8u * (stage + (e - b0)) + 7u);
        };
        auto tail_st = [&](uint32_t e, uint32_t v) {
            if (e >= WC_MAXN) wc_st16(B, 4u * (e - WC_MAXN) + 3u, v);
            else if (gstage) { const uint16_t t = (uint16_t)v; __builtin_memcpy(GB + 16u * (size_t)e + 14u, &t, 2); }
            else wc_st16(B, 8u * (stage + (e - b0)) + 7u, v);
        };
        const uint16_t* nin = W.nlist[cur]; uint16_t* nout = W.nlist[cur ^ 1u];
        auto clipped_id = [&](uint32_t i) -> uint32_t { return i < nCo ? b0 + i : (uint32_t)nin[i - nCo]; };
        const uint32_t cbase = carve(NI), ckm8 = 2u * carve((NI + 1u) / 2u);
        bool bad = false;
        WcRRState<2> st2;
        auto pfn = [&](uint32_t i) -> WcW4 { return i < nCo ? g.grec[b0 + i] : WcW4{0u, 0u, 0u, 0u}; };
        auto kfn = [&](uint32_t i, uint32_t& aux, const WcW4 wr) -> uint2 {
            uint32_t id; WcRec r;
            if (i < nCo)
            {
                stage_put(i, wr);
                id = b0 + i; r = WcRec{wr.a, wr.b, wr.c, wr.d};
            }
            else
            {
                id = nin[i - nCo];
                r = wc_rec(B, 8u * (id - WC_MAXN), true);
                if ((r.tail() & 0xFFu) != k) { wc_st8(B, ckm8 + i, 0u); aux = id << 8; return make_uint2(0u, 0u); }
            }
            uint32_t ee[7], tl[7];
#pragma unroll
            for (uint32_t q = 0; q < 7u; ++q) ee[q] = r.e(q);
#pragma unroll
            for (uint32_t q = 0; q < 7u; ++q) tl[q] = wc_ld16(B, ((ee[q] >= WC_MAXN ? 1u : 0u) & (ee[q] < WC_SENT ? 1u : 0u)) ? 4u * (ee[q] - WC_MAXN) + 3u : 3u);
            uint32_t km = 0;
#pragma unroll
            for (uint32_t q = 0; q < 7u; ++q)
            {
                const uint32_t isO = ee[q] < WC_MAXN ? 1u : 0u;
                const uint32_t kept = (isO & (ee[q] >= b1 ? 1u : 0u)) | ((isO ^ 1u) & (ee[q] < WC_SENT ? 1u : 0u) & ((tl[q] & 0xFFu) > k ? 1u : 0u));
                km |= kept << q;
            }
            {
                const uint32_t d01 = ((km & 3u) == 3u ? 1u : 0u) & (ee[0] == ee[1] ? 1u : 0u), d02 = ((km & 5u) == 5u ? 1u : 0u) & (ee[0] == ee[2] ? 1u : 0u),
                               d12 = ((km & 6u) == 6u ? 1u : 0u) & (ee[1] == ee[2] ? 1u : 0u);
                bad = bad | (((id >= WC_MAXN ? 1u : 0u) & (d01 | d02 | d12)) != 0u);
            }
            wc_st8(B, ckm8 + i, km | 0x80u);
            aux = km | 0x80u | (id << 8) | (((r.tail() >> 8) & 7u) << 24);
            return make_uint2(1u, (uint32_t)__builtin_popcount(km));
        };
        const uint2 nt = wc_rr_count<2>(W, sc, NI, st2, pfn, kfn, [&]() { WSTAMP(14); });
        WSTAMP(2);
        const uint32_t nC = nt.x, M = nt.y, nCn = nC - nCo, keepn = nl - nCn;
        const uint32_t dropAlive = SURTR_UNIFORM(W.hist[k]);
        const uint32_t dropKept = dropAlive - SURTR_UNIFORM(W.zhist[k]);
        if (nLive <= nC && dropKept == 0u)
        {
            if (nC == 0u) WC_RET(5);
            nLive = 0; break;
        }
        if (nC == 0u)
        {
            if (nLive + dropAlive < 4u) { nLive = 0; break; }
            continue;
        }
        if (M > 4095u || keepn + M > LT::kNL || nfree + nCn > LT::kNL) WC_RET(9);
        const uint32_t bmw = (M + 31u) / 32u;
        if (4u * rtop + 3u * M + 2u * bmw + 2u * nl + nCn + 72u > ltop) { if (tid == 0u && atomicAdd(&why[20], 1u) == 3u) { why[21] = n; why[22] = k; why[23] = rtop; why[24] = M; why[25] = nC; why[26] = nl; why[27] = ltop; why[28] = nfree; } WC_RET(10); }
        const uint32_t src = carve(M), srcid = carve(M), wst = carve(M), nd = carve(2u * nl), bm = carve(2u * bmw), clist = carve(nCn);
        const uint32_t fromf = nfree < M ? nfree : M, fromt = M - fromf, fh0 = fhead, fpush = fhead + nfree, tbase = rtop;
        {
            const uint32_t room = ltop / 4u > rtop ? ltop / 4u - rtop : 0u;
            if (fromt > room || rtop + fromt > capPool) { if (tid == 0u && atomicAdd(&why[20], 1u) == 3u) { why[21] = n; why[22] = k; why[23] = rtop; why[24] = M; why[25] = nC; why[26] = nl; why[27] = ltop; why[28] = nfree; } WC_RET(16); }
            rtop += fromt;
            fhead += fromf; if (fhead >= LT::kNL) fhead -= LT::kNL;
            nfree = nfree - fromf + nCn;
        }
        auto fring = [&](uint32_t at) -> uint32_t { return at >= LT::kNL ? at - LT::kNL : at; };
        auto xof = [&](uint32_t t) -> uint32_t { return WC_MAXN + (t < fromf ? (uint32_t)W.freel[fring(fh0 + t)] : tbase + (t - fromf)); };
        for (uint32_t q = tid; q < bmw; q += G) wc_st32(B, bm + 2u * q, 0u);
        WSTAMP(3);
        WCOUNT(18, 1); WCOUNT(19, nC); WCOUNT(20, M); WCOUNT(21, nl);
#ifdef SURTR_STAMP
        if (tid == 0u) { const unsigned long long need = 2ull * (4u * rtop + (8u * LT::kNR - ltop)); if (need > W.ph[31]) W.ph[31] = need; if (k >= 2u && need > W.ph[29]) W.ph[29] = need; }
#endif
        auto kfn2 = [&](uint32_t i, uint32_t& aux) -> uint2 {
            const uint32_t id = clipped_id(i), km = wc_ld8(B, ckm8 + i);
            if (!(km & 0x80u)) { aux = id << 8; return make_uint2(0u, 0u); }
            aux = km | (id << 8) | (((tail_ld(id) >> 8) & 7u) << 24);
            return make_uint2(1u, (uint32_t)__builtin_popcount(km & 0x7Fu));
        };
        wc_rr_place<2>(W, sc, NI, st2, kfn2, [&](uint32_t i, uint32_t xc, uint32_t xm, uint2 c, uint32_t aux) {
            const uint32_t km = aux & 0x7Fu, id = (aux >> 8) & 0xFFFFu, len = aux >> 24;
            if (!c.x) { nout[i - xc] = (uint16_t)id; return; }
            wc_st16(B, cbase + i, xm);
            tail_st(id, 0x8000u | (len << 12) | i);
            if (i >= nCo) { W.freel[fring(fpush + (xc - nCo))] = (uint16_t)(id - WC_MAXN); wc_st16(B, clist + (xc - nCo), i); }
            uint32_t t = xm;
            for (uint32_t m = km; m; m &= m - 1u, ++t) { wc_st16(B, src + t, i | ((uint32_t)__builtin_ctz(m) << 12)); wc_st16(B, srcid + t, id); }
        });
        cur ^= 1u;
        WSTAMP(15);
        __syncthreads();
        WSTAMP(4);
        const uint32_t nref = nLive + (k ? SURTR_UNIFORM(W.hist[k - 1u]) : dropTotal) + M;
        bool fail = false;
        auto walk = [&](uint32_t& cv, uint32_t& pcv, uint32_t& p, WcRec& rc, uint32_t& steps, const uint32_t limit, const bool jump) -> uint32_t {
            while (true)
            {
                if (jump && p == 0u && pcv >= nCo)
                {
                    const uint32_t a = wc_ld32(B, nd + 2u * (pcv - nCo)), jx = a & 0xFFFFu;
                    if (jx != pcv) { pcv = jx; cv = clipped_id(jx); steps += a >> 16; rc = rec_of(cv); }
                }
                const uint32_t kmc = wc_ld8(B, ckm8 + pcv);
                if ((kmc >> p) & 1u) return wc_ld16(B, cbase + pcv) + (uint32_t)__builtin_popcount(kmc & ((1u << p) - 1u));
                if (steps >= limit) return WC_NONE;
                const uint32_t e = rc.e(p);
                if (((e >= WC_SENT ? 1u : 0u) | ((e < WC_MAXN ? 1u : 0u) & ((e < b0 ? 1u : 0u) | (e >= b1 ? 1u : 0u))) | (steps + 2u >= nref ? 1u : 0u)) != 0u)
                { SURTR_DBG("  wc walk: sentinel / not clipped / bound e=%u steps=%u nref=%u k=%u\n", e, steps, nref, k); fail = true; return WC_NONE; }
                ++steps;
                const WcRec re = rec_of(e);
                const uint32_t te = re.tail();
                if (!(te & 0x8000u)) { SURTR_DBG("  wc walk: vertex %u not clipped now (tail %x) k=%u\n", e, te, k); fail = true; return WC_NONE; }
                const uint32_t le = (te >> 12) & 7u, q = re.find(cv, le);
                if (q >= le) { SURTR_DBG("  wc walk: no way back k=%u\n", k); fail = true; return WC_NONE; }
                p = q ? q - 1u : le - 1u; cv = e; pcv = te & 0xFFFu; rc = re;
            }
        };
        auto arrive = [&](uint32_t t, uint32_t end) {
            wc_st16(B, wst + t, 0xFFFFu);
            uint32_t* word = (uint32_t*)(void*)(B + 2u * (size_t)(bm + 2u * (end >> 5)));
            const uint32_t before = atomicOr(word, 1u << (end & 31u));
            if (((end == t ? 1u : 0u) | ((before >> (end & 31u)) & 1u)) != 0u) { SURTR_DBG("  wc walk: ends on itself / second arrival t=%u end=%u k=%u\n", t, end, k); fail = true; }
            const uint32_t X = xof(t), Z = xof(end);
            wc_st16(B, 4u * (Z - WC_MAXN), X);
            wc_st16(B, 4u * (X - WC_MAXN) + 1u, Z);
        };
        bool paused = false;
        uint32_t myz0 = 0, myz1 = 0;
        uint16_t* nnow = W.nlist[cur];
        for (uint32_t t = tid; t < M; t += G)
        {
            const uint32_t s = wc_ld16(B, src + t);
            const uint32_t v = wc_ld16(B, srcid + t), j = s >> 12;
            uint32_t pcv = s & 0xFFFu, cv = v;
            WcRec rc = rec_of(cv);
            const uint32_t u = rc.e(j);
            const float4 pa = *(v < WC_MAXN ? g.gpos + v : g.cpos + (v - WC_MAXN));
            const float4 pb = *(u < WC_MAXN ? g.gpos + u : g.cpos + (u - WC_MAXN));
            WcW4 wru = WcW4{0u, 0u, 0u, 0u};
            if (u < WC_MAXN) wru = g.grec[u];
            const uint32_t lv = (rc.tail() >> 12) & 7u;
            uint32_t p = j ? j - 1u : lv - 1u, steps = 0;
            const uint32_t end = walk(cv, pcv, p, rc, steps, walk0, false);
            const uint32_t X = xof(t), ux = X - WC_MAXN;
            const float sa = plane_dist(pl, pa.x, pa.y, pa.z), sb = plane_dist(pl, pb.x, pb.y, pb.z);
            const float inv = 1.f / (sb - sa);
            const float nx = (pa.x * sb - pb.x * sa) * inv, ny = (pa.y * sb - pb.y * sa) * inv, nz = (pa.z * sb - pb.z * sa) * inv;
            g.cpos[ux] = make_float4(nx, ny, nz, 0.f);
            const uint32_t f = planes_first_cut<SURTR_PLANE_CHUNK>(W.planes, k + 1u, F, nx, ny, nz,
                                                                   [&](uint32_t q) { if (q < 32u) myz0 |= 1u << q; else myz1 |= 1u << (q - 32u); });
            wc_st32(B, 4u * ux + 2u, u | ((f | (3u << 8)) << 16));
            nnow[keepn + t] = (uint16_t)X;
            const WcRec ru = u < WC_MAXN ? WcRec{wru.a, wru.b, wru.c, wru.d} : wc_rec(B, 8u * (u - WC_MAXN), true);
            const uint32_t tu = ru.tail(), qu = ru.find(v, (tu >> 8) & 7u);
            if ((tu & 0x8000u) || qu >= ((tu >> 8) & 7u)) { SURTR_DBG("  wc patch: kept end does not link the clipped vertex k=%u\n", k); fail = true; }
            else if (u < WC_MAXN) { const uint16_t xv = (uint16_t)X; __builtin_memcpy(GB + 16u * (size_t)u + 2u * qu, &xv, 2); }
            else wc_st16(B, 4u * (u - WC_MAXN) + qu, X);
            if (end != WC_NONE) arrive(t, end);
            else { wc_st16(B, wst + t, pcv | (p << 12)); paused = true; }
        }
        const bool anyPaused = wc_any(W, ac, paused, 0u);
        WSTAMP(5);
        if (anyPaused)
        {
            WCOUNT(24, 1);
            for (uint32_t ci = tid; ci < nCn; ci += G)
            {
                const uint32_t i = wc_ld16(B, clist + ci);
                const uint32_t c = clipped_id(i);
                const WcRec r = rec_of(c);
                const uint32_t e0 = r.e(0u);
                uint32_t nx = i, d = 0;
                if (!(wc_ld8(B, ckm8 + i) & 1u) && e0 >= WC_MAXN && e0 < WC_SENT)
                {
                    const WcRec r0 = rec_of(e0);
                    const uint32_t t0 = r0.tail();
                    if ((t0 & 0x8000u) && r0.find(c, (t0 >> 12) & 7u) == 1u) { nx = t0 & 0xFFFu; d = 1u; }
                }
                wc_st32(B, nd + 2u * (i - nCo), nx | (d << 16));
            }
            __syncthreads();
            for (uint32_t round = 0; round < 12u; ++round)
            {
                bool ch = false;
                for (uint32_t ci = tid; ci < nCn; ci += G)
                {
                    const uint32_t i = wc_ld16(B, clist + ci);
                    const uint32_t a = wc_ld32(B, nd + 2u * (i - nCo)), j1 = a & 0xFFFFu;
                    if (j1 == i) continue;
                    const uint32_t b2 = wc_ld32(B, nd + 2u * (j1 - nCo)), j2 = b2 & 0xFFFFu;
                    if (j2 == j1) continue;
                    const uint32_t b3 = wc_ld32(B, nd + 2u * (j2 - nCo)), j3 = b3 & 0xFFFFu;
                    wc_st32(B, nd + 2u * (i - nCo), j3 | (((a >> 16) + (b2 >> 16) + (j3 != j2 ? (b3 >> 16) : 0u)) << 16));
                    ch = true;
                }
                if (!wc_any(W, ac, ch, 0u)) break;
            }
            WSTAMP(6);
            for (uint32_t t = tid; t < M; t += G)
            {
                const uint32_t ws = wc_ld16(B, wst + t);
                if (ws == 0xFFFFu) continue;
                uint32_t pcv = ws & 0xFFFu, cv = clipped_id(pcv), p = ws >> 12, steps = walk0;
                WcRec rc = rec_of(cv);
                const uint32_t end = walk(cv, pcv, p, rc, steps, 0xFFFFFFFFu, true);
                if (end != WC_NONE) arrive(t, end);
                else fail = true;
#ifdef SURTR_STAMP
                atomicAdd(&g_wstamp[22], (unsigned long long)steps); atomicMax(&g_wstamp[23], (unsigned long long)steps);
#endif
            }
            WSTAMP(7);
        }
        if (myz0) atomicOr(&W.zm[0], myz0);
        if (myz1) atomicOr(&W.zm[1], myz1);
        if (wc_any(W, ac, fail || bad, 1u)) WC_RET(11);
        WSTAMP(8);
        zmask |= (unsigned long long)SURTR_UNIFORM(W.zm[0]) | ((unsigned long long)SURTR_UNIFORM(W.zm[1]) << 32);
        nLive = nLive - nC + M; nl = keepn + M;
        WSTAMP(9);
#ifdef SURTR_STAMP
        if (tid == 0u) { int c = 0; while (c < 7 && (32u << c) < NI) ++c; atomicAdd(&g_wplane[2 * c], 1ull); atomicAdd(&g_wplane[2 * c + 1], __builtin_readcyclecounter() - pl_t0); }
#endif
        if (nLive + dropAlive < 4u) { nLive = 0; break; }
    }
    __syncthreads();
    out.nl = nl; out.nLive = nLive; out.rtop = rtop; out.cur = cur;
    ctr.ac = ac; ctr.sc = sc;
    return 0;
}

template <class LT, class AR, class PR>
__device__ __attribute__((always_inline)) inline int wc_park(LT& W, const uint32_t F, const uint32_t n, const WcOut o, const WcGlob g,
                                                             const AR& A, PR& rec, WcCtr& ctr, uint32_t* __restrict__ why)
{
    const uint32_t tid = threadIdx.x, G = group_size(), lane = lane_id();
    unsigned char* B = W.U;
    const uint32_t bN = SURTR_UNIFORM(W.bst[F]);
    const uint32_t nOn = n - bN, nA = nOn + o.nl;
    const uint16_t* nlist = W.nlist[o.cur];
    uint32_t ac = ctr.ac, sc = ctr.sc;
    if (nA != o.nLive || nA >= 4096u) WC_RET(12);
    uint32_t ltop = 8u * LT::kNR;
    auto carve = [&](uint32_t cnt16) -> uint32_t { ltop -= (cnt16 + 7u) & ~7u; return ltop; };
    if (4u * o.rtop + 5u * (nA + 8u) > ltop) WC_RET(13);
    const uint32_t clen = carve(nA), coff = carve(nA), lab = carve(nA), local = carve(nA), olo = carve(nA);
    auto idof = [&](uint32_t i) -> uint32_t { return i < nOn ? bN + i : (uint32_t)nlist[i - nOn]; };
    auto recof = [&](uint32_t id) -> WcRec { if (id < WC_MAXN) { const WcW4 wr = g.grec[id]; return WcRec{wr.a, wr.b, wr.c, wr.d}; } return wc_rec(B, 8u * (id - WC_MAXN), true); };
    for (uint32_t i = tid; i < o.nl; i += G) wc_st16(B, 4u * ((uint32_t)nlist[i] - WC_MAXN) + 3u, 0x4000u | (nOn + i));
    WSTAMP_DECL;
    auto lenfn = [&](uint32_t i) -> uint2 { return make_uint2(i < nOn ? (g.grec[bN + i].d >> 24) & 7u : 3u, 0u); };
    const uint32_t H = wc_scan(W, sc, nA, lenfn, lenfn, [&](uint32_t i, uint32_t xo, uint32_t) {
        wc_st16(B, clen + i, lenfn(i).x); wc_st16(B, coff + i, xo); wc_st16(B, lab + i, i); }).x;
    if (H >= 0xFFFFu || 4u * o.rtop + H + 16u > ltop) WC_RET(14);
    const uint32_t cring = carve(H);
    __syncthreads();
    WSTAMP(10);
    bool odd = false;
    for (uint32_t i = tid; i < nA; i += G)
    {
        const WcRec r = recof(idof(i));
        const uint32_t off = wc_ld16(B, coff + i), len = wc_ld16(B, clen + i);
        for (uint32_t q = 0; q < len; ++q)
        {
            const uint32_t e = r.e(q);
            uint32_t rk = 0;
            if (e < WC_MAXN) { if (e < bN || e >= n) odd = true; else rk = e - bN; }
            else if (e >= WC_SENT) odd = true;
            else { const uint32_t te = wc_ld16(B, 4u * (e - WC_MAXN) + 3u); if ((te & 0xC000u) != 0x4000u) odd = true; rk = te & 0xFFFu; }
            if (rk >= nA) { odd = true; rk = 0; }
            wc_st16(B, cring + off + q, rk);
        }
    }
    if (wc_any(W, ac, odd)) WC_RET(15);
    WSTAMP(11);
    while (true)
    {
        bool ch = false;
        for (uint32_t i = tid; i < nA; i += G)
        {
            const uint32_t mine = wc_ld16(B, lab + i), off = wc_ld16(B, coff + i), len = wc_ld16(B, clen + i);
            uint32_t m = mine;
            for (uint32_t q = 0; q < len; ++q) { const uint32_t l2 = wc_ld16(B, lab + wc_ld16(B, cring + off + q)); m = l2 < m ? l2 : m; }
            const uint32_t mm = wc_ld16(B, lab + m);
            m = mm < m ? mm : m;
            if (m < mine) { wc_st16(B, lab + i, m); ch = true; }
        }
        if (!wc_any(W, ac, ch)) break;
    }
    WSTAMP(12);
    auto rootfn = [&](uint32_t i) -> uint2 { return make_uint2(wc_ld16(B, lab + i) == i ? 1u : 0u, 0u); };
    const uint32_t ni = wc_scan(W, sc, nA, rootfn, rootfn, [&](uint32_t, uint32_t, uint32_t) {}).x;
    __syncthreads();
    if (tid == 0u) { W.misc[0] = atomicAdd(&A.cursors[CUR_V], nA); W.misc[1] = atomicAdd(&A.cursors[CUR_H], H); W.misc[2] = atomicAdd(&A.cursors[CUR_ISL], ni); }
    __syncthreads();
    const uint32_t voff = W.misc[0], hoff = W.misc[1], ioff = W.misc[2];
    ctr.ac = ac; ctr.sc = sc;
    if ((uint64_t)voff + nA > A.capV || (uint64_t)hoff + H > A.capH || (uint64_t)ioff + ni > A.capIsl) return SURTR_E_CAPACITY;
    uint32_t vbase = 0, hbase = 0, root = 0;
    for (uint32_t t = 0; t < ni; ++t)
    {
        while (root < nA)
        {
            const uint32_t i = root + lane;
            const unsigned long long m = __ballot(i < nA && wc_ld16(B, lab + i) == i);
            if (m) { root += (uint32_t)__builtin_ctzll(m); break; }
            root += SURTR_LANES;
        }
        auto infn = [&](uint32_t i) -> uint2 { const bool in = wc_ld16(B, lab + i) == root; return make_uint2(in ? 1u : 0u, in ? wc_ld16(B, clen + i) : 0u); };
        const uint2 tt = wc_scan(W, sc, nA, infn, infn, [&](uint32_t i, uint32_t lv, uint32_t lh) {
            if (wc_ld16(B, lab + i) != root) return;
            wc_st16(B, local + i, lv); wc_st16(B, olo + i, lh);
            const size_t dv = (size_t)voff + vbase + lv;
            const uint32_t id = idof(i);
            const float4 p = id < WC_MAXN ? g.gpos[id] : g.cpos[id - WC_MAXN];
            A.pos[3u * dv] = p.x; A.pos[3u * dv + 1u] = p.y; A.pos[3u * dv + 2u] = p.z;
            A.llen[dv] = wc_ld16(B, clen + i); A.loff[dv] = hoff + hbase + lh;
        });
        if (tid == 0u) A.isl[ioff + t] = tt;
        __syncthreads();
        for (uint32_t i = tid; i < nA; i += G)
        {
            if (wc_ld16(B, lab + i) != root) continue;
            const uint32_t off = wc_ld16(B, coff + i), len = wc_ld16(B, clen + i);
            int32_t* d = A.nbr + (size_t)hoff + hbase + wc_ld16(B, olo + i);
            for (uint32_t q = 0; q < len; ++q) d[q] = (int32_t)wc_ld16(B, local + wc_ld16(B, cring + off + q));
        }
        vbase += tt.x; hbase += tt.y; root += 1u;
        __syncthreads();
    }
    ctr.sc = sc;
    rec.mv_off = voff; rec.mv_n = nA; rec.mh_off = hoff; rec.mh_n = H; rec.ni = ni; rec.isl_off = ioff;
    WSTAMP(13);
    return 0;
}

}
```

Before: 1.256 million.

## Run small clip planes on a single wave and skip empty plane scans

```diff
diff --git a/surtr_amd/csrc/prep_sorted.h b/surtr_amd/csrc/prep_sorted.h
--- a/surtr_amd/csrc/prep_sorted.h
+++ b/surtr_amd/csrc/prep_sorted.h
@@ -487,6 +487,7 @@
     for (uint32_t k = tid; k < F; k += group_size()) { W.hist[k] = hist[k]; W.zhist[k] = zhist[k]; }
     for (uint32_t k = tid; k <= F + 1u; k += group_size()) W.bst[k] = bst[k];
     if (tid == 0u) { W.zm[0] = 0u; W.zm[1] = 0u; for (int q = 0; q < 6; ++q) (&W.fl[0][0])[q] = 0u; }
+    if constexpr (LT::kSolo) for (uint32_t k = tid; k < WC_MAXF + 4u; k += group_size()) W.ccnt[k] = 0u;
     __syncthreads();
     WSTAMP(1);
     WCOUNT(16, 1); WCOUNT(17, n);
diff --git a/surtr_amd/csrc/surtr_ctx.h b/surtr_amd/csrc/surtr_ctx.h
--- a/surtr_amd/csrc/surtr_ctx.h
+++ b/surtr_amd/csrc/surtr_ctx.h
@@ -107,7 +107,10 @@
     CUR_CATCH_CLIPPED = 94,
     CUR_UNREFITTED = 95,
     CUR_WC_WHY = 96,
+    CUR_WC_SOLO_PLANES = 114,
+    CUR_WC_SOLO_STRETCHES = 115,
     CUR_Q_CONVEX2 = 125,
+    CUR_WC_SKIPPED = 126,
     CUR_STATS_WORDS = 128,
     CUR_HO_PUSHED = 146,
     CUR_HO_STARTED = 147,
diff --git a/surtr_amd/csrc/surtr_hip.hip b/surtr_amd/csrc/surtr_hip.hip
--- a/surtr_amd/csrc/surtr_hip.hip
+++ b/surtr_amd/csrc/surtr_hip.hip
@@ -1297,7 +1297,7 @@
                                                          const ScratchPool& pool, const Arena& A, const ImgArena& IA, PairRec* __restrict__ pairs,
                                                          const uint2* __restrict__ pair_list, const uint32_t* __restrict__ order,
                                                          uint32_t* __restrict__ horder, int cls_hi, int cls_lo, uint32_t qcur, uint32_t walk0,
-                                                         uint32_t* __restrict__ hlist, uint32_t cbase)
+                                                         uint32_t* __restrict__ hlist, uint32_t cbase, uint32_t solo_items = 0u)
 {
     WL& W = *reinterpret_cast<WL*>(lds_raw);
     GL& Gn = *reinterpret_cast<GL*>(lds_raw);
@@ -1353,7 +1353,7 @@
                 g = wc_glob(slot, pool.per_wg, rec.img_n, 2u * WL::kNR, fits);
                 if (fits) err = wc_load(W, im, F, g, zmask, ctr, A.cursors + CUR_WC_WHY);
             }
-            if (err == 0) err = wc_planes(W, F, rec.img_n, V - rec.img_n, zmask, g, 2u * WL::kNR, o, ctr, A.cursors + CUR_WC_WHY, walk0);
+            if (err == 0) err = wc_planes(W, F, rec.img_n, V - rec.img_n, zmask, g, 2u * WL::kNR, o, ctr, A.cursors + CUR_WC_WHY, walk0, solo_items);
             if (err == 0 && o.nLive != 0u) err = wc_park(W, F, rec.img_n, o, g, A, rec, ctr, A.cursors + CUR_WC_WHY);
 #ifdef SURTR_STAMP
             __syncthreads();
@@ -1421,16 +1421,16 @@
 #define SURTR_WR_MAIN 3072u
 #define SURTR_WNL_MAIN 3584u
 #endif
-typedef WcLdsT<SURTR_WR_MAIN, SURTR_WNL_MAIN, (SURTR_MAIN_THREADS / SURTR_LANES > SURTR_NWAVE ? SURTR_MAIN_THREADS / SURTR_LANES : SURTR_NWAVE), true> WcLdsMain;
+typedef WcLdsT<SURTR_WR_MAIN, SURTR_WNL_MAIN, (SURTR_MAIN_THREADS / SURTR_LANES > SURTR_NWAVE ? SURTR_MAIN_THREADS / SURTR_LANES : SURTR_NWAVE), true, true> WcLdsMain;
 __global__ __launch_bounds__(SURTR_MAIN_THREADS) __attribute__((amdgpu_waves_per_eu(SURTR_MAIN_THREADS > SURTR_WG ? 4 : 2, 4))) void k_clip_pairs_main(Pieces P, const float4* __restrict__ planes,
                                                          const uint32_t* __restrict__ plane_off, uint32_t cell_begin,
                                                          uint32_t n_pairs,
                                                          ScratchPool pool, Arena A, ImgArena IA, PairRec* __restrict__ pairs,
                                                          const uint2* __restrict__ pair_list, const uint32_t* __restrict__ order,
-                                                         uint32_t* __restrict__ hlist, uint32_t walk0)
+                                                         uint32_t* __restrict__ hlist, uint32_t walk0, uint32_t solo_items)
 {
     __shared__ alignas(16) unsigned char lds_raw[sizeof(WcLdsMain)];
-    clip_pairs_wave_body<WcLdsMain, WcLdsMain, false, true>(lds_raw, blockIdx.x, P, planes, plane_off, cell_begin, n_pairs, pool, A, IA, pairs, pair_list, order, nullptr, 11, 0, CUR_Q_CLIP, walk0, hlist, CUR_CLS_CLIP);
+    clip_pairs_wave_body<WcLdsMain, WcLdsMain, false, true>(lds_raw, blockIdx.x, P, planes, plane_off, cell_begin, n_pairs, pool, A, IA, pairs, pair_list, order, nullptr, 11, 0, CUR_Q_CLIP, walk0, hlist, CUR_CLS_CLIP, solo_items);
 }
 
 #define SURTR_H_TAKEN 0xFFFFFFFEu
@@ -3496,7 +3496,7 @@
     bool wave_on, split_on, use_half, front_par, both;
     bool cvx_lean;
     uint32_t rec_on;
-    uint32_t big_quota, big_n, walk0, n_catch, n_poll;
+    uint32_t big_quota, big_n, walk0, solo_items, n_catch, n_poll;
     uint32_t n_wg, n_wg_cvx, n_wg_lean, n_wg_cvx2, n_wg_prep, n_wg_big, n_wg_half, n_wg_retry, n_wg_sweep;
     uint32_t g_refit, g_faces, t_faces;
     hipStream_t st_cvx, st_main, st_bigk, st_refit;
@@ -3551,6 +3551,8 @@
     else if (n_pairs) pl.prep = k_prep_pairs;
     pl.walk0 = SURTR_WWALK0;
     if (const char* e = getenv("SURTR_WWALK0")) { const int v = atoi(e); if (v >= 0 && v <= 64) pl.walk0 = (uint32_t)v; }
+    pl.solo_items = SURTR_SOLO_ITEMS;
+    if (const char* e = getenv("SURTR_SOLO_ITEMS")) { const int v = atoi(e); if (v >= 0 && v <= 4095) pl.solo_items = (uint32_t)v; }
     pl.st_cvx = pl.front_par ? ctx->stream3 : ctx->stream;
     pl.st_main = pl.front_par ? ctx->stream : ctx->stream2;
     pl.st_bigk = pl.front_par ? ctx->stream2 : ctx->stream;
@@ -3699,7 +3701,7 @@
     if (wave) PROF_HIST_BEGIN(11, pl.st_main);
     if (split)
         hipLaunchKernelGGL(k_clip_pairs_main, dim3(pl.n_wg), dim3(SURTR_MAIN_THREADS), 0, pl.st_main, P, ctx->d_planes, ctx->d_plane_off, cell_begin, n_pairs,
-                           ctx->pool, ctx->arena, ctx->img, ctx->d_pairs, d_pair_list, order, ctx->d_hlist, pl.walk0);
+                           ctx->pool, ctx->arena, ctx->img, ctx->d_pairs, d_pair_list, order, ctx->d_hlist, pl.walk0, pl.solo_items);
     else if (wave)
         hipLaunchKernelGGL(k_clip_pairs_wave, dim3(pl.n_wg), dim3(SURTR_WG), 0, pl.st_main, P, ctx->d_planes, ctx->d_plane_off, cell_begin, n_pairs,
                            ctx->pool, ctx->arena, ctx->img, ctx->d_pairs, d_pair_list, order, horder, 13, 0, CUR_Q_CLIP, pl.walk0);
diff --git a/surtr_amd/csrc/wave_clip.h b/surtr_amd/csrc/wave_clip.h
--- a/surtr_amd/csrc/wave_clip.h
+++ b/surtr_amd/csrc/wave_clip.h
@@ -9,6 +9,9 @@
 #endif
 #ifndef SURTR_WWALK0
 #define SURTR_WWALK0 4u
+#endif
+#ifndef SURTR_SOLO_ITEMS
+#define SURTR_SOLO_ITEMS 128u
 #endif
 #define WC_MAXF 64u
 #define WC_MAXN 0x2000u
@@ -17,6 +20,19 @@
 #define WC_NONE 0xFFFFu
 #define WC_WHY_WORDS 29u
 static_assert(CUR_WC_WHY + WC_WHY_WORDS <= CUR_STATS_WORDS, "the why[] block ends inside what surtr_queue_stats copies out");
+#define WC_CNT_SOLO_PLANES 18u
+#define WC_CNT_SOLO_STRETCHES 19u
+#define WC_CNT_SKIPPED 30u
+static_assert(CUR_WC_WHY + WC_CNT_SOLO_PLANES == CUR_WC_SOLO_PLANES && CUR_WC_WHY + WC_CNT_SOLO_STRETCHES == CUR_WC_SOLO_STRETCHES &&
+              CUR_WC_WHY + WC_CNT_SKIPPED == CUR_WC_SKIPPED && CUR_WC_SKIPPED < CUR_STATS_WORDS, "the slot map names these words");
+#define WC_PLANE_NEXT 0
+#define WC_PLANE_DONE 1
+#define WC_PLANE_RET(site) return -(int)(site)
+#if SURTR_LANES == 64
+#define WC_WAVE_FENCE() __builtin_amdgcn_fence(__ATOMIC_ACQ_REL, "wavefront")
+#else
+#define WC_WAVE_FENCE() do { } while (0)
+#endif
 #define WC_RET(site) do { if (threadIdx.x == 0u) atomicAdd(&why[site], 1u); SURTR_DBG("record clip: pair handed on at site %d\n", site); return WC_BAIL; } while (0)
 #ifdef SURTR_STAMP
 __device__ unsigned long long g_wstamp[64];
@@ -78,10 +94,14 @@
     return r;
 }
 
-template <uint32_t NR, uint32_t NL = SURTR_WNL, uint32_t NW = SURTR_NWAVE, bool GSTAGE = (NR < SURTR_WR)>
-struct alignas(16) WcLdsT
+template <bool SOLO> struct WcSoloLds { };
+template <> struct WcSoloLds<true> { uint32_t ccnt[WC_MAXF + 4]; uint32_t back[2][12]; };
+#define WC_CC_SOLO (WC_MAXF + 1u)
+template <uint32_t NR, uint32_t NL = SURTR_WNL, uint32_t NW = SURTR_NWAVE, bool GSTAGE = (NR < SURTR_WR), bool SOLO = false>
+struct alignas(16) WcLdsT : WcSoloLds<SOLO>
 {
     static constexpr uint32_t kNR = NR, kNL = NL;
+    static constexpr bool kSolo = SOLO;
     static constexpr bool kGStage = GSTAGE;
     alignas(16) unsigned char U[16u * NR];
     float4 planes[WC_MAXF];
@@ -125,9 +145,20 @@
 struct WcOut { uint32_t nl, nLive, rtop, cur; };
 struct WcCtr { uint32_t ac, sc; };
 
-template <class LT>
-__device__ __forceinline__ bool wc_any(LT& W, uint32_t& c, bool pred, uint32_t slot = 0u)
-{
+template <bool SOLO>
+struct WcGrp
+{
+    static constexpr bool kSolo = SOLO;
+    __device__ __forceinline__ static uint32_t tid() { return SOLO ? lane_id() : threadIdx.x; }
+    __device__ __forceinline__ static uint32_t size() { return SOLO ? (uint32_t)SURTR_LANES : group_size(); }
+    __device__ __forceinline__ static uint32_t wave() { return SOLO ? 0u : wave_id(); }
+    __device__ __forceinline__ static uint32_t waves() { return SOLO ? 1u : group_waves(); }
+    __device__ __forceinline__ static void sync() { if (SOLO) WC_WAVE_FENCE(); else __syncthreads(); }
+};
+template <class GR, class LT>
+__device__ __forceinline__ bool wc_any(GR, LT& W, uint32_t& c, bool pred, uint32_t slot = 0u)
+{
+    if (GR::kSolo) return __ballot(pred) != 0ull;
     if (threadIdx.x == 0u) { W.fl[(c + 1u) % 3u][0] = 0u; W.fl[(c + 1u) % 3u][1] = 0u; }
     if (pred) W.fl[c % 3u][slot] = 1u;
     __syncthreads();
@@ -135,6 +166,8 @@
     ++c;
     return r;
 }
+template <class LT>
+__device__ __forceinline__ bool wc_any(LT& W, uint32_t& c, bool pred, uint32_t slot = 0u) { return wc_any(WcGrp<false>(), W, c, pred, slot); }
 
 template <class LT, class C1, class C2, class P>
 __device__ __forceinline__ uint2 wc_scan(LT& W, uint32_t& sc, uint32_t N, C1 count1, C2 count2, P place)
@@ -235,10 +268,10 @@
 }
 
 template <int NC> struct WcRRState { uint2 cc[NC], ss[NC], px; uint32_t ax[NC]; };
-template <int NC, class LT, class PF, class C, class M>
-__device__ __forceinline__ uint2 wc_rr_count(LT& W, uint32_t& sc, uint32_t N, WcRRState<NC>& st, PF pref, C count, M mid)
-{
-    const uint32_t lane = lane_id(), w = wave_id(), nw = group_waves();
+template <int NC, class GR, class LT, class PF, class C, class M>
+__device__ __forceinline__ uint2 wc_rr_count(GR, LT& W, uint32_t& sc, uint32_t N, WcRRState<NC>& st, PF pref, C count, M mid)
+{
+    const uint32_t lane = lane_id(), w = GR::wave(), nw = GR::waves();
     const uint32_t nb = (N + SURTR_LANES - 1u) >> SURTR_LSH;
     uint32_t* bs = W.bsum[sc & 1u];
     ++sc;
@@ -271,7 +304,7 @@
         if (lane == SURTR_LANES - 1u) { bs[2u * b] = s2.x; bs[2u * b + 1u] = s2.y; }
     }
     mid();
-    __syncthreads();
+    GR::sync();
     uint2 run = make_uint2(0u, 0u);
     st.px = make_uint2(0u, 0u);
     for (uint32_t c0 = 0; c0 < nb; c0 += SURTR_LANES)
@@ -291,10 +324,10 @@
     if (SURTR_LANES > 1u) return make_uint2(lane_bcast(st.px.x, b), lane_bcast(st.px.y, b));
     return make_uint2(bs[2u * b], bs[2u * b + 1u]);
 }
-template <int NC, class LT, class C, class P>
-__device__ __forceinline__ void wc_rr_place(LT& W, uint32_t sc_after, uint32_t N, WcRRState<NC>& st, C count, P place)
-{
-    const uint32_t lane = lane_id(), w = wave_id(), nw = group_waves();
+template <int NC, class GR, class LT, class C, class P>
+__device__ __forceinline__ void wc_rr_place(GR, LT& W, uint32_t sc_after, uint32_t N, WcRRState<NC>& st, C count, P place)
+{
+    const uint32_t lane = lane_id(), w = GR::wave(), nw = GR::waves();
     const uint32_t nb = (N + SURTR_LANES - 1u) >> SURTR_LSH;
     const uint32_t* bs = W.bsum[(sc_after - 1u) & 1u];
 #pragma unroll
@@ -333,6 +366,7 @@
     for (uint32_t k = tid; k < nw * (WC_MAXF + 2u); k += group_size()) (&W.wcnt[0][0])[k] = 0u;
     for (uint32_t k = tid; k < F; k += group_size()) { W.hist[k] = im.hist[k]; W.zhist[k] = im.zhist[k]; }
     if (tid == 0u) { W.zm[0] = 0u; W.zm[1] = 0u; for (int q = 0; q < 6; ++q) (&W.fl[0][0])[q] = 0u; }
+    if constexpr (LT::kSolo) for (uint32_t k = tid; k < WC_MAXF + 4u; k += group_size()) W.ccnt[k] = 0u;
     unsigned long long zm = 0ull;
     for (uint32_t k0 = 0; k0 < F; k0 += SURTR_LANES)
     {
@@ -422,30 +456,36 @@
 
 template <class LT>
 __device__ __attribute__((always_inline)) inline int wc_planes(LT& W, const uint32_t F, const uint32_t n, const uint32_t dropTotal, unsigned long long zmask,
-                                                               const WcGlob g, const uint32_t capPool, WcOut& out, WcCtr& ctr, uint32_t* __restrict__ why, const uint32_t walk0 = SURTR_WWALK0)
-{
-    const uint32_t tid = threadIdx.x, G = group_size();
+                                                               const WcGlob g, const uint32_t capPool, WcOut& out, WcCtr& ctr, uint32_t* __restrict__ why, const uint32_t walk0 = SURTR_WWALK0,
+                                                               const uint32_t soloT = 0u)
+{
     unsigned char* B = W.U;
     unsigned char* GB = (unsigned char*)g.grec;
     uint32_t rtop = 0, nl = 0, nLive = n, cur = 0, nfree = 0, fhead = 0;
     uint32_t ac = ctr.ac, sc = ctr.sc;
     out.nl = 0; out.nLive = 0; out.rtop = 0; out.cur = 0;
+    uint32_t k = 0, stretch = 0;
     WSTAMP_DECL;
-    for (uint32_t k = 0; k < F; ++k)
-    {
+    auto gstage_of = [&](uint32_t nCo, uint32_t NI) -> bool {
+        return LT::kGStage && nCo != 0u && 4u * rtop + 8u * nCo + NI + (NI + 1u) / 2u + 7u * NI + 3u * nl + 128u > 8u * LT::kNR;
+    };
+    auto plane = [&](auto grp) __attribute__((always_inline)) -> int
+    {
+        typedef decltype(grp) GR;
+        const uint32_t tid = GR::tid(), G = GR::size();
 #ifdef SURTR_STAMP
         const unsigned long long pl_t0 = __builtin_readcyclecounter();
 #endif
-        if ((zmask >> k) & 1ull) WC_RET(3);
+        if ((zmask >> k) & 1ull) WC_PLANE_RET(3);
         const float4 pl = W.planes[k];
         const uint32_t b0 = SURTR_UNIFORM(W.bst[k]), b1 = SURTR_UNIFORM(W.bst[k + 1u]);
         const uint32_t nCo = b1 - b0;
         uint32_t ltop = 8u * LT::kNR;
         auto carve = [&](uint32_t cnt16) -> uint32_t { ltop -= (cnt16 + 7u) & ~7u; return ltop; };
         const uint32_t NI = nCo + nl;
-        if (NI > 4095u) WC_RET(6);
-        const bool gstage = LT::kGStage && nCo != 0u && 4u * rtop + 8u * nCo + NI + (NI + 1u) / 2u + 7u * NI + 3u * nl + 128u > ltop;
-        if (4u * rtop + (gstage ? 0u : 8u * nCo) + NI + (NI + 1u) / 2u + 64u > ltop) WC_RET(4);
+        if (NI > 4095u) WC_PLANE_RET(6);
+        const bool gstage = gstage_of(nCo, NI);
+        if (4u * rtop + (gstage ? 0u : 8u * nCo) + NI + (NI + 1u) / 2u + 64u > ltop) WC_PLANE_RET(4);
         WCOUNT(26, gstage ? 1 : 0);
         const uint32_t stage = gstage ? 0u : carve(8u * nCo) / 8u;
         auto stage_put = [&](uint32_t i, const WcW4& wr) { if (!gstage) __builtin_memcpy(__builtin_assume_aligned(B + 16u * (size_t)(stage + i), 16), &wr, 16); };
@@ -505,29 +545,33 @@
             aux = km | 0x80u | (id << 8) | (((r.tail() >> 8) & 7u) << 24);
             return make_uint2(1u, (uint32_t)__builtin_popcount(km));
         };
-        const uint2 nt = wc_rr_count<2>(W, sc, NI, st2, pfn, kfn, [&]() { WSTAMP(14); });
+        bool scan = true;
+        if constexpr (LT::kSolo) scan = nCo + SURTR_UNIFORM(W.ccnt[k]) != 0u;
+        uint2 nt = make_uint2(0u, 0u);
+        if (scan) nt = wc_rr_count<2>(grp, W, sc, NI, st2, pfn, kfn, [&]() { WSTAMP(14); });
+        else if constexpr (LT::kSolo) { if (tid == 0u) W.ccnt[WC_CC_SOLO + 2u] += 1u; }
         WSTAMP(2);
         const uint32_t nC = nt.x, M = nt.y, nCn = nC - nCo, keepn = nl - nCn;
         const uint32_t dropAlive = SURTR_UNIFORM(W.hist[k]);
         const uint32_t dropKept = dropAlive - SURTR_UNIFORM(W.zhist[k]);
         if (nLive <= nC && dropKept == 0u)
         {
-            if (nC == 0u) WC_RET(5);
-            nLive = 0; break;
+            if (nC == 0u) WC_PLANE_RET(5);
+            nLive = 0; return WC_PLANE_DONE;
         }
         if (nC == 0u)
         {
-            if (nLive + dropAlive < 4u) { nLive = 0; break; }
-            continue;
-        }
-        if (M > 4095u || keepn + M > LT::kNL || nfree + nCn > LT::kNL) WC_RET(9);
+            if (nLive + dropAlive < 4u) { nLive = 0; return WC_PLANE_DONE; }
+            return WC_PLANE_NEXT;
+        }
+        if (M > 4095u || keepn + M > LT::kNL || nfree + nCn > LT::kNL) WC_PLANE_RET(9);
         const uint32_t bmw = (M + 31u) / 32u;
-        if (4u * rtop + 3u * M + 2u * bmw + 2u * nl + nCn + 72u > ltop) { if (tid == 0u && atomicAdd(&why[20], 1u) == 3u) { why[21] = n; why[22] = k; why[23] = rtop; why[24] = M; why[25] = nC; why[26] = nl; why[27] = ltop; why[28] = nfree; } WC_RET(10); }
+        if (4u * rtop + 3u * M + 2u * bmw + 2u * nl + nCn + 72u > ltop) { if (tid == 0u && atomicAdd(&why[20], 1u) == 3u) { why[21] = n; why[22] = k; why[23] = rtop; why[24] = M; why[25] = nC; why[26] = nl; why[27] = ltop; why[28] = nfree; } WC_PLANE_RET(10); }
         const uint32_t src = carve(M), srcid = carve(M), wst = carve(M), nd = carve(2u * nl), bm = carve(2u * bmw), clist = carve(nCn);
         const uint32_t fromf = nfree < M ? nfree : M, fromt = M - fromf, fh0 = fhead, fpush = fhead + nfree, tbase = rtop;
         {
             const uint32_t room = ltop / 4u > rtop ? ltop / 4u - rtop : 0u;
-            if (fromt > room || rtop + fromt > capPool) { if (tid == 0u && atomicAdd(&why[20], 1u) == 3u) { why[21] = n; why[22] = k; why[23] = rtop; why[24] = M; why[25] = nC; why[26] = nl; why[27] = ltop; why[28] = nfree; } WC_RET(16); }
+            if (fromt > room || rtop + fromt > capPool) { if (tid == 0u && atomicAdd(&why[20], 1u) == 3u) { why[21] = n; why[22] = k; why[23] = rtop; why[24] = M; why[25] = nC; why[26] = nl; why[27] = ltop; why[28] = nfree; } WC_PLANE_RET(16); }
             rtop += fromt;
             fhead += fromf; if (fhead >= LT::kNL) fhead -= LT::kNL;
             nfree = nfree - fromf + nCn;
@@ -546,7 +590,7 @@
             aux = km | (id << 8) | (((tail_ld(id) >> 8) & 7u) << 24);
             return make_uint2(1u, (uint32_t)__builtin_popcount(km & 0x7Fu));
         };
-        wc_rr_place<2>(W, sc, NI, st2, kfn2, [&](uint32_t i, uint32_t xc, uint32_t xm, uint2 c, uint32_t aux) {
+        wc_rr_place<2>(grp, W, sc, NI, st2, kfn2, [&](uint32_t i, uint32_t xc, uint32_t xm, uint2 c, uint32_t aux) {
             const uint32_t km = aux & 0x7Fu, id = (aux >> 8) & 0xFFFFu, len = aux >> 24;
             if (!c.x) { nout[i - xc] = (uint16_t)id; return; }
             wc_st16(B, cbase + i, xm);
@@ -557,7 +601,7 @@
         });
         cur ^= 1u;
         WSTAMP(15);
-        __syncthreads();
+        GR::sync();
         WSTAMP(4);
         const uint32_t nref = nLive + (k ? SURTR_UNIFORM(W.hist[k - 1u]) : dropTotal) + M;
         bool fail = false;
@@ -618,6 +662,7 @@
             const uint32_t f = planes_first_cut<SURTR_PLANE_CHUNK>(W.planes, k + 1u, F, nx, ny, nz,
                                                                    [&](uint32_t q) { if (q < 32u) myz0 |= 1u << q; else myz1 |= 1u << (q - 32u); });
             wc_st32(B, 4u * ux + 2u, u | ((f | (3u << 8)) << 16));
+            if constexpr (LT::kSolo) atomicAdd(&W.ccnt[f < WC_MAXF ? f : WC_MAXF], 1u);
             nnow[keepn + t] = (uint16_t)X;
             const WcRec ru = u < WC_MAXN ? WcRec{wru.a, wru.b, wru.c, wru.d} : wc_rec(B, 8u * (u - WC_MAXN), true);
             const uint32_t tu = ru.tail(), qu = ru.find(v, (tu >> 8) & 7u);
@@ -627,7 +672,7 @@
             if (end != WC_NONE) arrive(t, end);
             else { wc_st16(B, wst + t, pcv | (p << 12)); paused = true; }
         }
-        const bool anyPaused = wc_any(W, ac, paused, 0u);
+        const bool anyPaused = wc_any(grp, W, ac, paused, 0u);
         WSTAMP(5);
         if (anyPaused)
         {
@@ -647,7 +692,7 @@
                 }
                 wc_st32(B, nd + 2u * (i - nCo), nx | (d << 16));
             }
-            __syncthreads();
+            GR::sync();
             for (uint32_t round = 0; round < 12u; ++round)
             {
                 bool ch = false;
@@ -662,7 +707,7 @@
                     wc_st32(B, nd + 2u * (i - nCo), j3 | (((a >> 16) + (b2 >> 16) + (j3 != j2 ? (b3 >> 16) : 0u)) << 16));
                     ch = true;
                 }
-                if (!wc_any(W, ac, ch, 0u)) break;
+                if (!wc_any(grp, W, ac, ch, 0u)) break;
             }
             WSTAMP(6);
             for (uint32_t t = tid; t < M; t += G)
@@ -682,7 +727,7 @@
         }
         if (myz0) atomicOr(&W.zm[0], myz0);
         if (myz1) atomicOr(&W.zm[1], myz1);
-        if (wc_any(W, ac, fail || bad, 1u)) WC_RET(11);
+        if (wc_any(grp, W, ac, fail || bad, 1u)) WC_PLANE_RET(11);
         WSTAMP(8);
         zmask |= (unsigned long long)SURTR_UNIFORM(W.zm[0]) | ((unsigned long long)SURTR_UNIFORM(W.zm[1]) << 32);
         nLive = nLive - nC + M; nl = keepn + M;
@@ -690,9 +735,63 @@
 #ifdef SURTR_STAMP
         if (tid == 0u) { int c = 0; while (c < 7 && (32u << c) < NI) ++c; atomicAdd(&g_wplane[2 * c], 1ull); atomicAdd(&g_wplane[2 * c + 1], __builtin_readcyclecounter() - pl_t0); }
 #endif
-        if (nLive + dropAlive < 4u) { nLive = 0; break; }
+        if (nLive + dropAlive < 4u) { nLive = 0; return WC_PLANE_DONE; }
+        return WC_PLANE_NEXT;
+    };
+    auto count_out = [&]() {
+        if constexpr (LT::kSolo) if (threadIdx.x == 0u)
+        {
+            const uint32_t* cn = W.ccnt + WC_CC_SOLO;
+            if (cn[0]) { atomicAdd(&why[WC_CNT_SOLO_PLANES], cn[0]); atomicAdd(&why[WC_CNT_SOLO_STRETCHES], cn[1]); }
+            if (cn[2]) atomicAdd(&why[WC_CNT_SKIPPED], cn[2]);
+        }
+    };
+    auto small_plane = [&]() -> bool {
+        const uint32_t nCo = SURTR_UNIFORM(W.bst[k + 1u]) - SURTR_UNIFORM(W.bst[k]), NI = nCo + nl;
+        return soloT != 0u && NI <= soloT && !gstage_of(nCo, NI);
+    };
+    while (k < F)
+    {
+        int r = WC_PLANE_NEXT;
+        bool wide = true;
+        if constexpr (LT::kSolo) wide = !small_plane();
+        if (wide)
+        {
+            r = plane(WcGrp<false>());
+            if (r == WC_PLANE_NEXT) ++k;
+        }
+        else if constexpr (LT::kSolo)
+        {
+            uint32_t* back = W.back[stretch & 1u];
+            if (SURTR_UNIFORM(wave_id()) == 0u)
+            {
+                const uint32_t k0 = k;
+                do { r = plane(WcGrp<true>()); if (r == WC_PLANE_NEXT) ++k; } while (r == WC_PLANE_NEXT && k < F && small_plane());
+                if (lane_id() == 0u)
+                {
+                    back[0] = k; back[1] = rtop; back[2] = nl; back[3] = nLive; back[4] = cur; back[5] = nfree; back[6] = fhead;
+                    back[7] = (uint32_t)zmask; back[8] = (uint32_t)(zmask >> 32); back[9] = ac; back[10] = sc; back[11] = (uint32_t)r;
+                    W.ccnt[WC_CC_SOLO] += (k - k0) + (r == WC_PLANE_NEXT ? 0u : 1u); W.ccnt[WC_CC_SOLO + 1u] += 1u;
+                }
+            }
+            __syncthreads();
+            k = SURTR_UNIFORM(back[0]); rtop = SURTR_UNIFORM(back[1]); nl = SURTR_UNIFORM(back[2]); nLive = SURTR_UNIFORM(back[3]);
+            cur = SURTR_UNIFORM(back[4]); nfree = SURTR_UNIFORM(back[5]); fhead = SURTR_UNIFORM(back[6]);
+            zmask = (unsigned long long)SURTR_UNIFORM(back[7]) | ((unsigned long long)SURTR_UNIFORM(back[8]) << 32);
+            ac = SURTR_UNIFORM(back[9]); sc = SURTR_UNIFORM(back[10]); r = (int)SURTR_UNIFORM(back[11]);
+            ++stretch;
+        }
+        if (r < 0)
+        {
+            count_out();
+            if (threadIdx.x == 0u) atomicAdd(&why[-r], 1u);
+            SURTR_DBG("record clip: pair handed on at site %d\n", -r);
+            return WC_BAIL;
+        }
+        if (r == WC_PLANE_DONE) break;
     }
     __syncthreads();
+    count_out();
     out.nl = nl; out.nLive = nLive; out.rtop = rtop; out.cur = cur;
     ctr.ac = ac; ctr.sc = sc;
     return 0;
```

Result: no change. 1.249 million (-0.6%).
